# tachitachi/SR-WaveNet

Hardware: AMD Instinct MI355X
Metric: audio samples/sec (fwd+bwd) 30-layer teacher WaveNet (higher is better)
Workload: dtype bf16; 1 GPU; 30-layer teacher WaveNet (3x[1..512] dilations, 64 res / 256 skip ch, 256-way mu-law softmax), fwd+bwd+Adam, batch 8x16000 samples per GPU; global_batch=8, seq_len=16000, parallelism=dp1, launch=hipGraph

## Files before the change

include/srwn.h:

```cpp
#ifndef SRWN_H
#define SRWN_H
#include <stdint.h>

#ifdef __cplusplus
extern "C" {
#endif

#define SRWN_F32 0
#define SRWN_BF16 1

#define SRWN_E_DTYPE (-1)
#define SRWN_E_SHAPE (-2)
#define SRWN_E_NULL (-3)
#define SRWN_E_UNSUPPORTED (-4)

#define SRWN_PRO_NONE 0
#define SRWN_PRO_GATE 1
#define SRWN_EPI_NONE 0
#define SRWN_EPI_RELU 1
#define SRWN_EPI_MASK 2
#define SRWN_EPI_F32 4

int srwn_version(void);
const char* srwn_last_error(void);
// ... 80 lines not shown
                           int64_t y_row_stride, int32_t y_chunk_len, int64_t y_chunk_stride, int32_t cout_pad,
                           int32_t cout_valid, int64_t rows, int32_t dtype, void* stream);

int srwn_pw_linear_ksplit(const void* x, int64_t x_row_stride, int64_t x_chunk_stride, int32_t chunk_len, int32_t Cin,
                          const void* wpack, const float* bias, float* y_partials, int64_t y_row_stride,
                          int32_t cout_pad, int32_t cout_valid, int64_t rows, int32_t nsplit, int32_t dtype,
                          void* stream);

int64_t srwn_softmax_ce_partials(int64_t rows);
int srwn_head_softmax_ce(const void* x, int64_t x_row_stride, int32_t Cin, const void* wpack, const float* bias,
                         const int32_t* targets, float* loss_partials, void* dlogits, float* logits_out,
                         int32_t cout_pad, int32_t cout_valid, int64_t rows, float grad_scale, int32_t dtype,
                         void* stream);
int srwn_reduce_loss(const float* loss_partials, int64_t n, float scale, float* loss_out, void* stream);

int srwn_head_chain(const void* r0, const void* w1, const void* w2_perm, const void* w2T_perm, const void* w1T_perm,
                    const float* b1, const float* b2, const int32_t* targets, float* loss_partials, void* r1,
                    void* dlogits, void* da1, void* dtotal, int32_t S, int32_t cout_pad, int32_t cout_valid,
                    int64_t rows, float grad_scale, int32_t dtype, void* stream);

int srwn_residual_layer_bwd(const void* g_in, const void* df_up, const void* wconvT_up, void* g_out,
                            const void* wresT, const void* wskipT, const void* dtotal, const void* dcs,
                            const void* z, void* df_out, int32_t B, int32_t T, int32_t R, int32_t S, int32_t K,
                            int32_t dilation_up, int32_t has_up, int32_t has_down, int32_t dtype, void* stream);

int32_t srwn_wgrad_slabs(int64_t rows);
int srwn_wgrad(const void* in, int64_t in_batch_stride, int32_t cin, const void* dout, int64_t dout_batch_stride,
               int32_t cout, const void* cond, int64_t cond_batch_stride, int32_t cond_frames, int32_t pool_stride,
               int32_t cond_row_stride, const int32_t* shifts , int32_t nbatch, float* partials,
               float* bias_partials, int64_t rows, int32_t T, int32_t nslabs, int32_t pro, int32_t dtype,
               void* stream);
int srwn_reduce_partials(const float* partials, int32_t nslabs, int64_t n, int32_t nbatch, int32_t partials_batched,
                         float scale, float* out, int64_t out_batch_stride, void* stream);
#define SRWN_PARTIALS_F32 0
#define SRWN_PARTIALS_BLK16 1
#define SRWN_PARTIALS_SUM 2
typedef struct SrwnReduceJob {
  const void* partials; int32_t nslabs; int64_t n; int32_t nbatch; int32_t partials_batched; float scale;
  float* out; int64_t out_batch_stride;
  int32_t layout; int32_t blk_cols;
} SrwnReduceJob;
int srwn_reduce_partials_multi(const SrwnReduceJob* jobs, int32_t njobs, void* stream);

int srwn_add_frame_bias(void* x, const void* bias, int64_t bias_row_stride, int32_t B, int32_t T, int32_t C,
                        int32_t frames, int32_t pool_stride, int32_t dtype, void* stream);
int srwn_frame_sum(const void* g, void* out, int32_t B, int32_t T, int32_t C, int32_t frames, int32_t pool_stride,
                   int32_t dtype, void* stream);
int srwn_frame_sum_batched(const void* g, int64_t g_batch_stride, void* out, int64_t out_batch_stride, int32_t nbatch,
                           int32_t B, int32_t T, int32_t C, int32_t frames, int32_t pool_stride, float scale,
                           int32_t dtype, void* stream);

int srwn_adam_step(float* params, const float* grads, float* m, float* v, int64_t n, int64_t* step, float lr,
                   float beta1, float beta2, float eps, float grad_scale, void* stream);

int32_t srwn_time_mean_slabs(int32_t T);
int srwn_time_mean(const void* x, float* partials, float* out, int32_t B, int32_t T, int32_t C, int32_t dtype,
                   void* stream);
int srwn_pooled_head(const float* mean, const float* w2, const float* b2, const float* labels, float* probs,
                     float* loss, float* gw2, float* gb2, float* dmean, int32_t B, int32_t S, int32_t C,
                     int32_t ldw, void* stream);
int srwn_bcast_mask(const float* dmean, const void* r1, void* out, int32_t B, int32_t T, int32_t S, float scale,
                    int32_t dtype, void* stream);

int srwn_wavenet_layer_fwd(const void* x, const void* cond, const void* wconv, const void* wres, const float* bias_f,
                           const float* bias_g, const float* bias_r, void* h_out, void* z_out, void* s_out, void* c_out,
                           int32_t B, int32_t T, int32_t R, int32_t K, int32_t dilation, int32_t cond_frames,
                           int32_t pool_stride, int32_t cond_row_stride, int32_t dtype, void* stream);
int srwn_wavenet_layer_bwd(const void* g_in, const void* d_up, const void* wconvT_up, void* g_out, const void* wresT,
                           const void* wskipT, const void* dtotal, const void* dcs, const void* z, const void* s,
                           void* d_out, int32_t B, int32_t T, int32_t R, int32_t S, int32_t K, int32_t dilation_up,
                           int32_t has_up, int32_t has_down, int32_t dtype, void* stream);

int srwn_contrastive_head(const float* mean, const float* w2, const float* b2, const float* labels, float margin,
                          float* emb, float* dist, float* loss, float* gw2, float* gb2, float* dmean, int32_t rows,
                          int32_t S, int32_t D, int32_t ldw, void* stream);

int32_t srwn_wgrad256_slabs(int64_t rows, int32_t m_chunks);
int32_t srwn_wgrad_wide_slabs(int64_t rows, int32_t m_chunks, int32_t chunk_width);
int srwn_wgrad_wide(const void* a, int64_t a_chunk_stride, int64_t a_row_stride, int32_t m_chunks, int32_t chunk_width,
                    const void* d, int64_t d_row_stride, int32_t d_width, float* partials, float* bias_partials,
                    int64_t rows, int32_t nslabs, int32_t pro, int32_t dtype, void* stream);
int srwn_wgrad_wide_pair(const void* a0, const void* d0, float* partials0, float* bias_partials0, const void* a1,
                         const void* d1, float* partials1, float* bias_partials1, int64_t a_chunk_stride,
                         int64_t a_row_stride, int32_t m_chunks, int32_t chunk_width, int64_t d_row_stride,
                         int32_t d_width, int64_t rows, int32_t nslabs, int32_t pro, int32_t dtype, void* stream);
int srwn_wgrad256(const void* a, int64_t a_chunk_stride, int64_t a_row_stride, int32_t m_chunks, const void* d,
                  int64_t d_row_stride, float* partials, float* bias_partials, int64_t rows, int32_t nslabs,
                  int32_t pro, int32_t dtype, void* stream);

int srwn_skip_dgrad_all(const void* dtotal, const void* wskipT_all, void* dcs, int64_t dcs_layer_stride,
                        int32_t nlayers, int64_t rows, int32_t R, int32_t S, int32_t dtype, void* stream);

int srwn_wgrad_layers(const void* x, const void* z, const void* df, const void* g, int64_t layer_stride,
                      const void* cond, int64_t cond_layer_stride, int32_t cond_frames, int32_t pool_stride,
                      int32_t cond_row_stride, const int32_t* dilations, int32_t nlayers, float* part_f,
                      float* part_r, float* part_bf, float* part_br, int64_t rows, int32_t T, int32_t nslabs,
                      int32_t R, int32_t K, int32_t dtype, void* stream);

int32_t srwn_wgrad_skip_wt_slabs(const int32_t* st, const int32_t* seg_rows, int32_t nlayers, int32_t T);
int srwn_wgrad_skip_wt(const void* cT, int64_t wt_layer_stride, const int32_t* st, const int32_t* seg_rows,
                       int32_t nlayers, const void* d, int64_t d_row_stride, void* partials, float* bias_partials,
                       int32_t part16, int32_t nslabs, int32_t B, int32_t T, int32_t R, int32_t S, int32_t dtype,
                       void* stream);

int64_t srwn_generate_ring_elems(const int32_t* dilations, int32_t nlayers, int32_t R);
int srwn_generate(const void* wcr, const void* wskip, const void* w1, const void* w2, const float* bias_f,
// ... 323 lines not shown
```

sr-wavenet_amd/_lib.py:

```python
from __future__ import annotations

import ctypes as C
import numbers
import os

HERE = os.path.dirname(os.path.abspath(__file__))
LIB_PATH = os.path.join(HERE, "libsrwn.so")
_ALT_LIB = os.environ.get("SRWN_LIB_PATH")
if _ALT_LIB:
    LIB_PATH = _ALT_LIB

F32, BF16 = 0, 1
PRO_NONE, PRO_GATE = 0, 1
EPI_NONE, EPI_RELU, EPI_MASK, EPI_F32 = 0, 1, 2, 4

_p, _i32, _i64, _f32 = C.c_void_p, C.c_int32, C.c_int64, C.c_float


class SrwnGenSlot(C.Structure):
    _fields_ = [("t", C.c_int32), ("t_end", C.c_int32), ("seed", C.c_uint64)]


class SrwnSynthSlot(C.Structure):
    _fields_ = [("t", C.c_int64), ("t_end", C.c_int64)]
# ... 130 lines not shown
    "srwn_nc_encode_partials": (_i64, [_i32, _i32, _i32, _i32]),
    "srwn_nc_encode_frames": (C.c_int, [_p, _i64, _p, _p, _p, _p, _p, _i64, _p, _i64, _p, _p, _p, _p, _i32, _i32, _i32, _i32,
                                        _i32, _i32, _i32, _i32, _p]),
    "srwn_nc_encode_list_partials": (_i64, [_i32, _i32, _i32]),
    "srwn_nc_encode_frame_list": (C.c_int, [_p, _i32, _i32, _p, _i32, _p, _p, _p, _p, _p, _i64, _p, _i64, _p, _p, _p, _p,
                                            _i32, _i32, _i32, _i32, _i32, _p]),
    "srwn_audio_ring_put": (C.c_int, [_p, _i32, _i32, _p, _p, _p, _p, _p, _i32, _i32, _p]),
    "srwn_small_gemm": (C.c_int, [_p, _i64, _i32, _i64, _i32, _p, _i64, _i64, _i32, _i64, _p, _p, _i64, _i32, _i32,
                                  _i32, _i32, _i32, _p]),
    "srwn_small_wgrad": (C.c_int, [_p, _i64, _p, _i64, _p, _p, _i32, _i32, _i32, _f32, _p]),
    "srwn_mol_sample": (C.c_int, [_p, _i64, _i32, _p, _p, _p, _i64, _p]),
    "srwn_mol_loss_dx": (C.c_int, [_p, _i64, _p, _i32, _p, _p, _i64, _f32, _p]),
    "srwn_clamp": (C.c_int, [_p, _p, _i64, _f32, _f32, _p]),
    "srwn_clamp_bwd": (C.c_int, [_p, _p, _p, _i64, _f32, _f32, _p]),
    "srwn_flow_partials": (_i64, [_i64]),
    "srwn_flow_affine_fwd": (C.c_int, [_p, _p, _p, _p, _p, _p, _p, _i64, _i32, _i32, _p]),
    "srwn_flow_affine_bwd": (C.c_int, [_p, _p, _p, _p, _p, _f32, _p, _p, _p, _i64, _i32, _i32, _p]),
    "srwn_flow_stream_in": (C.c_int, [_p, _i64, _p, _p, _p, _p, _i32, _i32, _i64, _p, _i64, _i32, _i32, _i32, _i32, _i32,
                                      _i32, _p, _p]),
    "srwn_residual_group_fwd_stream": (C.c_int, [_p, _i64, _p, _i64, _i32, _p, _p, _p, _p, _p, _i32, _i32, _i32, _p, _i32,
                                                 _i32, _i32, _i32, _i32, _i32, _i32, _p, _p]),
    "srwn_flow_stream_out": (C.c_int, [_p, _i64, _p, _p, _p, _p, _i64, _p, _i32, _p, _i32, _i32, _i32, _i32, _i32, _i32, _p,
                                       _i32, _p]),
    "srwn_logistic_noise": (C.c_int, [_p, _i64, _p, _p, _p, _i32, _i32, _p]),
    "srwn_logistic_from_bits": (C.c_int, [_p, _p, _i64, _p]),
    "srwn_logistic_noise_slots": (C.c_int, [_p, _i64, _p, _p, _p, _i32, _i32, _p]),
    "srwn_flow_stream_in_slots": (C.c_int, [_p, _i64, _p, _p, _p, _p, _i32, _i32, _i64, _p, _i64, _i32, _i32, _i32, _i32,
                                            _i32, _i32, _p, _p]),
    "srwn_residual_group_fwd_stream_slots": (C.c_int, [_p, _i64, _p, _i64, _i32, _p, _p, _p, _p, _p, _i32, _i32, _i32, _p,
                                                       _i32, _i32, _i32, _i32, _i32, _i32, _i32, _p, _p]),
    "srwn_flow_stream_out_slots": (C.c_int, [_p, _i64, _p, _p, _p, _p, _i64, _p, _i32, _p, _i32, _i32, _i32, _i32, _i32,
                                             _i32, _p, _p, _i32, _p]),
    "srwn_flow_stream_reset_slots": (C.c_int, [_p, _i32, _p, _i32, _i64, _p, _i32, _i32, _i32, _i32, _p]),
    "srwn_cond_ring_feed": (C.c_int, [_p, _i64, _i64, _i32, _p, _p, _p, _i32, _i32, _i32, _i32, _p, _p, _p, _i32, _i32,
                                      _i32, _p]),
    "srwn_causal_conv1d_dgrad": (C.c_int, [_p, _p, _p, _i32, _i32, _i32, _i32, _i32, _i32, _i32, _i32, _f32, _i32, _p]),
    "srwn_stft_frames": (_i32, [_i32]),
    "srwn_stft_power": (C.c_int, [_p, _p, _p, _p, _i32, _i32, _p]),
    "srwn_power_loss": (C.c_int, [_p, _p, _i64, _f32, _f32, _p, _p, _p]),
    "srwn_stft_power_bwd": (C.c_int, [_p, _p, _p, _i32, _i32, _i32, _p]),
    "srwn_axpy_dev": (C.c_int, [_p, _p, _p, _f32, _i64, _p]),
    "srwn_sumsq_partials": (_i64, [_i64]),
    "srwn_sumsq": (C.c_int, [_p, _i64, _p, _p]),
    "srwn_clip_scale": (C.c_int, [_p, _i64, _f32, _f32, _p, _p]),
    "srwn_adam_step_scaled": (C.c_int, [_p, _p, _p, _p, _i64, _p, _f32, _f32, _f32, _f32, _p, _i32, _p]),
}

for _n in SAMPLED:
    SIGNATURES[_n + "_sampled"] = (SIGNATURES[_n][0], SIGNATURES[_n][1] + [_p])
del _n
for _n in ("srwn_generate", "srwn_generate16"):
    SIGNATURES[_n + "_mol_live_sampled"] = SIGNATURES[_n + "_mol_resume_sampled"]
del _n
SIGNATURES["srwn_cond_ring_scatter"] = (C.c_int, [_p, _i64, _p, _i64, _i32, _i32, _i64, _i32, _i32, _i32, _p])

_lib = None
BINDING = None


def signature_hash() -> str:
    import hashlib
    txt = ";".join("%s:%s:%s" % (n, r.__name__, ",".join(a.__name__ for a in args)) for n, (r, args) in SIGNATURES.items())
    return hashlib.sha256(txt.encode()).hexdigest()[:16]


def _address(a):
    if a is None:
        return 0
    if isinstance(a, (int, float)):
        return a
    if isinstance(a, numbers.Integral):
        return int(a)
    if isinstance(a, numbers.Real):
        return float(a)
    if isinstance(a, C.Array):
        return C.addressof(a)
    if isinstance(a, C._SimpleCData):
        return a.value or 0
    if hasattr(a, "_obj"):
        return C.addressof(a._obj)
    raise TypeError("cannot pass %r through the C-ABI" % (a,))


class _PybindLib:

    def __init__(self, mod, keepalive):
        self._keepalive = keepalive
        for name in SIGNATURES:
            fn = getattr(mod, name)
            setattr(self, name, (lambda f: lambda *args: f(*[_address(a) for a in args]))(fn))


def pybind_path() -> str:
    import sysconfig
    return os.path.join(HERE, "_srwn_pyb" + sysconfig.get_config_var("EXT_SUFFIX"))


def bind(kind: str):
    if kind not in ("pybind11", "ctypes"):
        raise RuntimeError("SRWN_BINDING=%s: pybind11 or ctypes" % kind)
    if not os.path.exists(LIB_PATH):
        raise RuntimeError(
            "libsrwn.so not found at %s: build it with `python sr-wavenet_amd/build.py` "
            "(there is no CPU fallback for the product path)" % LIB_PATH)
    if _ALT_LIB:
        kind = "ctypes"
    else:
# ... 51 lines not shown
```

sr-wavenet_amd/csrc/srwn_bwd.hip:

```cpp
#include <cstdlib>
#include "srwn_common.h"
#include "srwn_host.h"
#include "../../include/srwn.h"

using namespace srwn;

struct LayerBwdArgs {
  const void* g_in;
  const void* df_up;
  const void* wconvT;
  void* g_out;
  const void* wresT;
  const void* wskipT;
  const void* dtotal;
  const void* dcs;
  const void* z;
  void* df_out;
  int Tlen, dil_up, S, ntb, ntiles;
};

template <typename T> struct Raw4;
template <> struct Raw4<bf16_t> {
  typedef bf16x4 type;
  static __device__ __forceinline__ type load(const bf16_t* p) { return *reinterpret_cast<const bf16x4*>(p); }
  static __device__ __forceinline__ float get(const type& v, int e) { return (float)v[e]; }
};
template <> struct Raw4<float> {
  typedef f32x4 type;
  static __device__ __forceinline__ type load(const float* p) { return *reinterpret_cast<const f32x4*>(p); }
  static __device__ __forceinline__ float get(const type& v, int e) { return v[e]; }
};

template <typename T, int RT, int K, int UPM, bool GIN, bool DOWN, int SK>
__global__ __launch_bounds__(256, (sizeof(T) == 2 && SK != 0) ? 2 : 1) void layer_bwd_kernel(LayerBwdArgs a) {
  constexpr int R = 32 * RT, KS = R / 16;
  constexpr bool UP = UPM == 1, HAVEG = UPM != 0, DCS = SK == 1, LEGACY = SK == 0;
  typedef typename Raw4<T>::type raw4;
  const int KSS = a.S / 16;
  extern __shared__ __attribute__((aligned(16))) char smem[];
  Frag<T>* lds_conv = reinterpret_cast<Frag<T>*>(smem);
  Frag<T>* lds_res = lds_conv + (UP ? RT * K * KS * 64 : 0);
  Frag<T>* lds_skip = lds_res + ((HAVEG && DOWN) ? RT * KS * 64 : 0);
  const int lane = threadIdx.x & 63, wave = __builtin_amdgcn_readfirstlane(threadIdx.x >> 6);
  constexpr bool ROWS = sizeof(T) == 2 && !LEGACY;
  constexpr int LS = RowStage<T>::stride(R), VEC = RowStage<T>::VEC;
  constexpr int LPR = R / VEC, RPI = 64 / LPR, NI = 32 / RPI;
  T* stage_all = reinterpret_cast<T*>(lds_skip + ((DOWN && LEGACY) ? RT * KSS * 64 : 0));
  T* stage = stage_all + wave * (32 * LS);
  if (UP) lds_dma_copy(a.wconvT, lds_conv, RT * K * KS * 64 * (int)sizeof(Frag<T>), wave, lane, 4);
  if (HAVEG && DOWN) lds_dma_copy(a.wresT, lds_res, RT * KS * 64 * (int)sizeof(Frag<T>), wave, lane, 4);
  if (DOWN && LEGACY) lds_dma_copy(a.wskipT, lds_skip, RT * KSS * 64 * (int)sizeof(Frag<T>), wave, lane, 4);

  const int col = lane & 31, half = lane >> 5;
  struct Tile {
    raw4 gin[RT][4];
// ... 534 lines not shown
}

__global__ void reduce_partials_kernel(const float* __restrict__ partials, int nslabs, int64_t n, int nbatch,
                                       int part_batch_mul, float scale, float* __restrict__ out,
                                       int64_t out_batch_stride) {
  const int64_t i = (int64_t)blockIdx.x * blockDim.x + threadIdx.x;
  const int l = blockIdx.y;
  if (i >= n || l >= nbatch) return;
  const float* p = partials + (int64_t)l * part_batch_mul * nslabs * n + i;
  double s = 0.0;
  int k = 0;
  for (; k + 8 <= nslabs; k += 8) {
    float v[8];
#pragma unroll
    for (int j = 0; j < 8; ++j) v[j] = p[(int64_t)(k + j) * n];
#pragma unroll
    for (int j = 0; j < 8; ++j) s += (double)v[j];
  }
  for (; k < nslabs; ++k) s += (double)p[(int64_t)k * n];
  out[(int64_t)l * out_batch_stride + i] = (float)(s * (double)scale);
}

__global__ __launch_bounds__(256) void reduce_partials_wide_kernel(const float* __restrict__ partials, int nslabs,
                                                                   int64_t n, int nbatch, int part_batch_mul,
                                                                   float scale, float* __restrict__ out,
                                                                   int64_t out_batch_stride) {
  const int64_t i = (int64_t)blockIdx.x * 16 + (threadIdx.x >> 4);
  const int l = blockIdx.y, sub = threadIdx.x & 15;
  double s = 0.0;
  if (i < n) {
    const float* p = partials + (int64_t)l * part_batch_mul * nslabs * n + i;
    int k = sub;
    for (; k + 16 * 7 < nslabs; k += 16 * 8) {
      float v[8];
#pragma unroll
      for (int j = 0; j < 8; ++j) v[j] = p[(int64_t)(k + 16 * j) * n];
#pragma unroll
      for (int j = 0; j < 8; ++j) s += (double)v[j];
    }
    for (; k < nslabs; k += 16) s += (double)p[(int64_t)k * n];
  }
#pragma unroll
  for (int w = 8; w > 0; w >>= 1) s += __shfl_xor(s, w, 64);
  if (i < n && sub == 0) out[(int64_t)l * out_batch_stride + i] = (float)(s * (double)scale);
}

#define SRWN_NT_LOAD(p) __builtin_nontemporal_load(p)
constexpr int kRpMaxJobs = 16;
struct RpJob {
  const float* partials; float* out; int64_t n; int64_t out_batch_stride;
  int nslabs, nbatch, part_batch_mul; float scale; int wide; unsigned blocks_x, block0;
  int blk_cols;
  int sg;
};
struct RpMulti { RpJob j[kRpMaxJobs]; int njobs; };

__global__ __launch_bounds__(256) void reduce_partials_multi_kernel(RpMulti m) {
  int k = 0;
  while (k + 1 < m.njobs && blockIdx.x >= m.j[k + 1].block0) ++k;
  const RpJob& job = m.j[k];
  const unsigned b = blockIdx.x - job.block0;
  const unsigned bx = b % job.blocks_x;
  const int l = (int)(b / job.blocks_x);
  const int nslabs = job.nslabs;
  const int64_t n = job.n;
  if (job.wide == 4) {
    __shared__ double red[256];
    const int64_t total = (int64_t)nslabs * n;
    double acc = 0.0;
    for (int64_t i = threadIdx.x; i < total; i += 256) acc += (double)job.partials[i];
    red[threadIdx.x] = acc;
    __syncthreads();
    for (int w = 128; w > 0; w >>= 1) {
      if ((int)threadIdx.x < w) red[threadIdx.x] += red[threadIdx.x + w];
      __syncthreads();
    }
    if (threadIdx.x == 0) job.out[0] = (float)(red[0] * (double)job.scale);
    return;
  }
  if (job.wide == 3) {
    __shared__ double red[256 * 8];
    const int sg = job.sg, qpb = 256 / sg;
    const int qi = (int)threadIdx.x % qpb, g = (int)threadIdx.x / qpb;
    const int64_t q = (int64_t)bx * qpb + qi;
    const bool live = q * 8 < n;
    const int per = nslabs / sg, k0 = g * per, k1 = (g == sg - 1) ? nslabs : k0 + per;
    double s[8];
#pragma unroll
    for (int e = 0; e < 8; ++e) s[e] = 0.0;
    if (live) {
      const bf16_t* p = reinterpret_cast<const bf16_t*>(job.partials) + (int64_t)l * job.part_batch_mul * nslabs * n + q * 8;
      int k = k0;
      for (; k + 8 <= k1; k += 8) {
        srwn::bf16x8 v[8];
#pragma unroll
        for (int j = 0; j < 8; ++j) v[j] = SRWN_NT_LOAD(reinterpret_cast<const srwn::bf16x8*>(p + (int64_t)(k + j) * n));
#pragma unroll
        for (int j = 0; j < 8; ++j)
#pragma unroll
          for (int e = 0; e < 8; ++e) s[e] += (double)(float)v[j][e];
      }
      for (; k < k1; ++k) {
        const srwn::bf16x8 v = *reinterpret_cast<const srwn::bf16x8*>(p + (int64_t)k * n);
#pragma unroll
        for (int e = 0; e < 8; ++e) s[e] += (double)(float)v[e];
      }
    }
    if (sg > 1) {
      if (g > 0) {
#pragma unroll
        for (int e = 0; e < 8; ++e) red[(g * qpb + qi) * 8 + e] = s[e];
      }
      __syncthreads();
      if (g > 0) return;
      for (int gg = 1; gg < sg; ++gg) {
#pragma unroll
        for (int e = 0; e < 8; ++e) s[e] += red[(gg * qpb + qi) * 8 + e];
      }
    }
    if (!live) return;
    const int64_t blk = q >> 5;
    const int pr = (int)(q & 31);
    const int nib = job.blk_cols / 16;
    const int lane = 2 * pr;
    const int64_t row0 = 16 * (blk / nib) + 4 * (lane >> 4);
    const int col = 16 * (int)(blk % nib) + (lane & 15);
    const double sc = (double)job.scale;
    float* o = job.out + (int64_t)l * job.out_batch_stride + row0 * job.blk_cols + col;
#pragma unroll
    for (int rr = 0; rr < 4; ++rr) {
      typedef float f2 __attribute__((ext_vector_type(2)));
      *reinterpret_cast<f2*>(o + (int64_t)rr * job.blk_cols) = f2{(float)(s[rr] * sc), (float)(s[4 + rr] * sc)};
    }
  } else if (job.wide == 1) {
    const int64_t i = (int64_t)bx * 16 + (threadIdx.x >> 4);
    const int sub = threadIdx.x & 15;
    double s = 0.0;
    if (i < n) {
      const float* p = job.partials + (int64_t)l * job.part_batch_mul * nslabs * n + i;
      int q = sub;
      for (; q + 16 * 7 < nslabs; q += 16 * 8) {
        float v[8];
#pragma unroll
        for (int j = 0; j < 8; ++j) v[j] = p[(int64_t)(q + 16 * j) * n];
#pragma unroll
        for (int j = 0; j < 8; ++j) s += (double)v[j];
      }
      for (; q < nslabs; q += 16) s += (double)p[(int64_t)q * n];
    }
#pragma unroll
    for (int w = 8; w > 0; w >>= 1) s += __shfl_xor(s, w, 64);
    if (i < n && sub == 0) job.out[(int64_t)l * job.out_batch_stride + i] = (float)(s * (double)job.scale);
  } else if (job.wide == 2) {
    const int64_t i = ((int64_t)bx * 256 + threadIdx.x) * 4;
    if (i >= n) return;
    const float* p = job.partials + (int64_t)l * job.part_batch_mul * nslabs * n + i;
    double s0 = 0.0, s1 = 0.0, s2 = 0.0, s3 = 0.0;
    int q = 0;
    for (; q + 8 <= nslabs; q += 8) {
      srwn::f32x4 v[8];
#pragma unroll
      for (int j = 0; j < 8; ++j) v[j] = SRWN_NT_LOAD(reinterpret_cast<const srwn::f32x4*>(p + (int64_t)(q + j) * n));
#pragma unroll
      for (int j = 0; j < 8; ++j) { s0 += (double)v[j][0]; s1 += (double)v[j][1]; s2 += (double)v[j][2]; s3 += (double)v[j][3]; }
    }
    for (; q < nslabs; ++q) {
      const srwn::f32x4 v = *reinterpret_cast<const srwn::f32x4*>(p + (int64_t)q * n);
      s0 += (double)v[0]; s1 += (double)v[1]; s2 += (double)v[2]; s3 += (double)v[3];
    }
    const double sc = (double)job.scale;
    *reinterpret_cast<srwn::f32x4*>(job.out + (int64_t)l * job.out_batch_stride + i) =
        srwn::f32x4{(float)(s0 * sc), (float)(s1 * sc), (float)(s2 * sc), (float)(s3 * sc)};
  } else {
    const int64_t i = (int64_t)bx * 256 + threadIdx.x;
    if (i >= n) return;
    const float* p = job.partials + (int64_t)l * job.part_batch_mul * nslabs * n + i;
    double s = 0.0;
    int q = 0;
    for (; q + 8 <= nslabs; q += 8) {
      float v[8];
#pragma unroll
      for (int j = 0; j < 8; ++j) v[j] = p[(int64_t)(q + j) * n];
#pragma unroll
      for (int j = 0; j < 8; ++j) s += (double)v[j];
    }
    for (; q < nslabs; ++q) s += (double)p[(int64_t)q * n];
    job.out[(int64_t)l * job.out_batch_stride + i] = (float)(s * (double)job.scale);
  }
}

extern "C" int srwn_reduce_partials_multi(const SrwnReduceJob* jobs, int32_t njobs, void* stream) {
  if (njobs == 0) return 0;
  if (!jobs) return set_error(SRWN_E_NULL, "reduce_partials_multi: null pointer");
  if (njobs < 0 || njobs > kRpMaxJobs) return set_error(SRWN_E_SHAPE, "reduce_partials_multi: %d jobs (1..%d)", njobs, kRpMaxJobs);
  RpMulti m;
  m.njobs = 0;
  uint64_t blocks = 0;
  for (int k = 0; k < njobs; ++k) {
    const SrwnReduceJob& q = jobs[k];
    if (q.n == 0 || q.nbatch == 0) continue;
    if (!q.partials || !q.out) return set_error(SRWN_E_NULL, "reduce_partials_multi: job %d: null pointer", k);
    if (q.nslabs < 1 || q.n < 0 || q.nbatch < 0 || q.nbatch > 65535)
      return set_error(SRWN_E_SHAPE, "reduce_partials_multi: job %d: nslabs=%d n=%lld nbatch=%d", k, q.nslabs, (long long)q.n, q.nbatch);
    RpJob& j = m.j[m.njobs++];
    j.partials = reinterpret_cast<const float*>(q.partials); j.out = q.out; j.n = q.n; j.out_batch_stride = q.out_batch_stride;
    j.nslabs = q.nslabs; j.nbatch = q.nbatch; j.part_batch_mul = q.partials_batched ? 1 : 0; j.scale = q.scale;
    j.wide = (q.n <= 4096 && q.nslabs >= 32) ? 1 : 0;
    if (q.nslabs >= 128 && q.n >= 1024 && q.n % 4 == 0 && q.out_batch_stride % 4 == 0 &&
        (reinterpret_cast<uintptr_t>(q.partials) | reinterpret_cast<uintptr_t>(q.out)) % 16 == 0)
      j.wide = 2;
    j.blk_cols = 0; j.sg = 1;
    if (q.layout == SRWN_PARTIALS_BLK16) {
      if (q.blk_cols < 16 || q.blk_cols % 16 || q.n % (16 * (int64_t)q.blk_cols) || q.out_batch_stride % 2 ||
          (reinterpret_cast<uintptr_t>(q.partials) % 16) || (reinterpret_cast<uintptr_t>(q.out) % 8))
        return set_error(SRWN_E_SHAPE, "reduce_partials_multi: job %d: BLK16 layout needs n = rows*blk_cols in whole 16 x 16 blocks (n=%lld, blk_cols=%d)", k, (long long)q.n, q.blk_cols);
      j.wide = 3; j.blk_cols = q.blk_cols;
      j.sg = 1;
      while (j.sg < 8 && q.nslabs / (2 * j.sg) >= 8 && (q.n / 8) * (int64_t)q.nbatch * j.sg < (int64_t)256 * 16 * 64) j.sg *= 2;
    } else if (q.layout == SRWN_PARTIALS_SUM) {
      if (q.nbatch != 1) return set_error(SRWN_E_SHAPE, "reduce_partials_multi: job %d: SUM layout has one output", k);
      j.wide = 4;
    } else if (q.layout != SRWN_PARTIALS_F32) {
      return set_error(SRWN_E_UNSUPPORTED, "reduce_partials_multi: job %d: layout %d", k, q.layout);
    }
    j.blocks_x = (unsigned)(j.wide == 4 ? 1 : j.wide == 3 ? (q.n / 8 + 256 / j.sg - 1) / (256 / j.sg) : j.wide == 2 ? (q.n / 4 + 255) / 256 : j.wide ? (q.n + 15) / 16 : (q.n + 255) / 256);
    j.block0 = (unsigned)blocks;
    blocks += (uint64_t)j.blocks_x * (uint64_t)q.nbatch;
    if (blocks > 0x7fffffffull) return set_error(SRWN_E_SHAPE, "reduce_partials_multi: grid too large");
  }
  if (m.njobs == 0) return 0;
  hipLaunchKernelGGL(reduce_partials_multi_kernel, dim3((unsigned)blocks), dim3(256), 0, (hipStream_t)stream, m);
  return check_launch("reduce_partials_multi");
}

extern "C" int srwn_reduce_partials(const float* partials, int32_t nslabs, int64_t n, int32_t nbatch,
                                    int32_t partials_batched, float scale, float* out, int64_t out_batch_stride,
                                    void* stream) {
  if (n == 0 || nbatch == 0) return 0;
  if (!partials || !out) return set_error(SRWN_E_NULL, "reduce_partials: null pointer");
  if (nslabs < 1 || n < 0 || nbatch < 0 || nbatch > 65535) return set_error(SRWN_E_SHAPE, "reduce_partials: nslabs=%d n=%lld nbatch=%d", nslabs, (long long)n, nbatch);
  if (n <= 4096 && nslabs >= 32) {
    dim3 grid((unsigned)((n + 15) / 16), (unsigned)nbatch), block(256);
    hipLaunchKernelGGL(reduce_partials_wide_kernel, grid, block, 0, (hipStream_t)stream, partials, nslabs, n, nbatch,
                       partials_batched ? 1 : 0, scale, out, out_batch_stride);
    return check_launch("reduce_partials");
  }
  dim3 grid((unsigned)((n + 255) / 256), (unsigned)nbatch), block(256);
  hipLaunchKernelGGL(reduce_partials_kernel, grid, block, 0, (hipStream_t)stream, partials, nslabs, n, nbatch,
                     partials_batched ? 1 : 0, scale, out, out_batch_stride);
  return check_launch("reduce_partials");
}

template <typename T> struct FsRow;
template <> struct FsRow<bf16_t> {
  static __device__ __forceinline__ void load(const bf16_t* p, float (&v)[8]) {
    const bf16x8 r = *reinterpret_cast<const bf16x8*>(p);
#pragma unroll
    for (int j = 0; j < 8; ++j) v[j] = (float)r[j];
  }
};
template <> struct FsRow<float> {
  static __device__ __forceinline__ void load(const float* p, float (&v)[8]) {
    const f32x4 a = *reinterpret_cast<const f32x4*>(p), b = *reinterpret_cast<const f32x4*>(p + 4);
#pragma unroll
    for (int j = 0; j < 4; ++j) { v[j] = a[j]; v[4 + j] = b[j]; }
  }
};

template <typename T, int C>
__global__ __launch_bounds__(256) void frame_sum_kernel(const T* __restrict__ g, int64_t g_batch_stride,
                                                        T* __restrict__ out, int64_t out_batch_stride, int Tlen,
                                                        int frames, int pool, float scale) {
  constexpr int LPR = C / 8, RPI = 256 / LPR;
  __shared__ float red[256 * 8];
  const int e = blockIdx.x, b = blockIdx.y, l = blockIdx.z;
  const int sub = threadIdx.x % LPR, rloc = threadIdx.x / LPR;
  const int t0 = e * pool;
  const int t1 = min(t0 + pool, Tlen);
  const T* src = g + (int64_t)l * g_batch_stride + (int64_t)b * Tlen * C + 8 * sub;
  float acc[8] = {0, 0, 0, 0, 0, 0, 0, 0};
  for (int t = t0 + rloc; t < t1; t += RPI) {
    float v[8];
    FsRow<T>::load(src + (int64_t)t * C, v);
#pragma unroll
    for (int j = 0; j < 8; ++j) acc[j] += v[j];
// ... 108 lines not shown
```

sr-wavenet_amd/csrc/srwn_opt.hip:

```cpp
#include "srwn_common.h"
#include "srwn_host.h"
#include "../../include/srwn.h"

using namespace srwn;

constexpr int kAdamBlocks = 256;
static unsigned adam_grid(int64_t n) {
  const int64_t b = (n + 1023) / 1024;
  return (unsigned)(b < kAdamBlocks ? b : kAdamBlocks);
}
static int adam_vec(const void* a, const void* b, const void* c, const void* d) {
  return ((((uintptr_t)a) | ((uintptr_t)b) | ((uintptr_t)c) | ((uintptr_t)d)) & 15) == 0;
}

__global__ __launch_bounds__(256) void adam_step_kernel(float* __restrict__ theta, const float* __restrict__ g,
                                                        float* __restrict__ m, float* __restrict__ v, int64_t n,
                                                        int64_t* step, int tick, float lr, float b1, float b2,
                                                        float eps, float grad_scale,
                                                        const float* __restrict__ scale_dev, int vec) {
  __shared__ float s_lr;
  __shared__ int s_t;
  if (threadIdx.x == 0) {
    const int count = __hip_atomic_load(reinterpret_cast<int*>(step), __ATOMIC_RELAXED, __HIP_MEMORY_SCOPE_AGENT);
    s_t = count + (tick ? 1 : 0);
    const double t = (double)s_t;
    s_lr = (float)((double)lr * sqrt(1.0 - pow((double)b2, t)) / (1.0 - pow((double)b1, t)));
  }
  __syncthreads();
  const float lr_t = s_lr;
  if (scale_dev) grad_scale *= scale_dev[0];
  auto one = [&](float gi, float& mi, float& vi, float& th) {
    gi *= grad_scale;
    mi = b1 * mi + (1.0f - b1) * gi;
    vi = b2 * vi + (1.0f - b2) * gi * gi;
    th -= lr_t * mi / (sqrtf(vi) + eps);
  };
  for (int64_t i0 = ((int64_t)blockIdx.x * blockDim.x + threadIdx.x) * 4; i0 < n; i0 += (int64_t)gridDim.x * blockDim.x * 4) {
    if (vec && i0 + 4 <= n) {
      typedef float f4 __attribute__((ext_vector_type(4)));
      f4 gg = *reinterpret_cast<const f4*>(g + i0), mm = *reinterpret_cast<f4*>(m + i0), vv = *reinterpret_cast<f4*>(v + i0),
         tt = *reinterpret_cast<f4*>(theta + i0);
#pragma unroll
      for (int j = 0; j < 4; ++j) { float a = mm[j], b = vv[j], c = tt[j]; one(gg[j], a, b, c); mm[j] = a; vv[j] = b; tt[j] = c; }
      *reinterpret_cast<f4*>(m + i0) = mm;
      *reinterpret_cast<f4*>(v + i0) = vv;
      *reinterpret_cast<f4*>(theta + i0) = tt;
    } else {
      for (int64_t i = i0; i < n && i < i0 + 4; ++i) one(g[i], m[i], v[i], theta[i]);
    }
  }
  if (tick && threadIdx.x == 0) {
    unsigned* arrived = reinterpret_cast<unsigned*>(step) + 1;
    const unsigned prev = __hip_atomic_fetch_add(arrived, 1u, __ATOMIC_RELAXED, __HIP_MEMORY_SCOPE_AGENT);
    if (prev == gridDim.x - 1)
      __hip_atomic_store(step, (int64_t)s_t, __ATOMIC_RELAXED, __HIP_MEMORY_SCOPE_AGENT);
  }
}

extern "C" int srwn_adam_step(float* params, const float* grads, float* m, float* v, int64_t n, int64_t* step,
                              float lr, float beta1, float beta2, float eps, float grad_scale, void* stream) {
  if (n == 0) return 0;
  if (!params || !grads || !m || !v || !step) return set_error(SRWN_E_NULL, "adam_step: null pointer");
  if (n < 0) return set_error(SRWN_E_SHAPE, "adam_step: n=%lld", (long long)n);
  hipStream_t st = (hipStream_t)stream;
  hipLaunchKernelGGL(adam_step_kernel, dim3(adam_grid(n)), dim3(256), 0, st, params, grads, m, v, n,
                     step, 1, lr, beta1, beta2, eps, grad_scale, (const float*)nullptr, adam_vec(params, grads, m, v));
  return check_launch("adam_step");
}

extern "C" int srwn_adam_step_scaled(float* params, const float* grads, float* m, float* v, int64_t n, int64_t* step,
                                     float lr, float beta1, float beta2, float eps, const float* grad_scale_dev,
                                     int32_t tick, void* stream) {
  if (n == 0) return 0;
  if (!params || !grads || !m || !v || !step || !grad_scale_dev)
    return set_error(SRWN_E_NULL, "adam_step_scaled: null pointer");
  if (n < 0) return set_error(SRWN_E_SHAPE, "adam_step_scaled: n=%lld", (long long)n);
  hipStream_t st = (hipStream_t)stream;
  hipLaunchKernelGGL(adam_step_kernel, dim3(adam_grid(n)), dim3(256), 0, st, params, grads, m, v, n,
                     step, tick ? 1 : 0, lr, beta1, beta2, eps, 1.0f, grad_scale_dev, adam_vec(params, grads, m, v));
  return check_launch("adam_step_scaled");
}
```

sr-wavenet_amd/csrc/srwn_pybind.cpp:

```cpp
#include <pybind11/pybind11.h>
#include <cstdint>
#include "../../include/srwn.h"
namespace py = pybind11;
namespace {
struct P {
  std::uintptr_t v;
  template <class T> operator T*() const { return reinterpret_cast<T*>(v); }
};
}

PYBIND11_MODULE(_srwn_pyb, m) {
  m.doc() = "pybind11 binding of libsrwn.so (include/srwn.h)";
  m.attr("SIGNATURE_HASH") = "921a0d5f5da475ed";
  m.def("srwn_version", []() { return srwn_version(); });
  m.def("srwn_last_error", []() { const char* r = srwn_last_error(); return py::bytes(r ? r : ""); });
  m.def("srwn_mu_law_encode", [](std::uintptr_t a0, std::uintptr_t a1, int64_t a2, int a3, std::uintptr_t a4) { return srwn_mu_law_encode(P{a0}, P{a1}, a2, a3, P{a4}); });
  m.def("srwn_mu_law_decode", [](std::uintptr_t a0, std::uintptr_t a1, int64_t a2, int a3, std::uintptr_t a4) { return srwn_mu_law_decode(P{a0}, P{a1}, a2, a3, P{a4}); });
  m.def("srwn_pack_a_index", [](std::uintptr_t a0, int a1, int a2, int a3, int a4, int a5, int a6, int a7, int a8, int a9, int a10, std::uintptr_t a11) { return srwn_pack_a_index(P{a0}, a1, a2, a3, a4, a5, a6, a7, a8, a9, a10, P{a11}); });
  m.def("srwn_pack_gather", [](std::uintptr_t a0, std::uintptr_t a1, std::uintptr_t a2, int64_t a3, int a4, std::uintptr_t a5) { return srwn_pack_gather(P{a0}, P{a1}, P{a2}, a3, a4, P{a5}); });
  m.def("srwn_pack_gather_rowsum", [](std::uintptr_t a0, std::uintptr_t a1, std::uintptr_t a2, int64_t a3, int a4, std::uintptr_t a5, int a6, int a7, std::uintptr_t a8, std::uintptr_t a9) { return srwn_pack_gather_rowsum(P{a0}, P{a1}, P{a2}, a3, a4, P{a5}, a6, a7, P{a8}, P{a9}); });
  m.def("srwn_causal_conv1d_fwd", [](std::uintptr_t a0, std::uintptr_t a1, std::uintptr_t a2, std::uintptr_t a3, int a4, int a5, int a6, int a7, int a8, int a9, int a10, int a11, std::uintptr_t a12) { return srwn_causal_conv1d_fwd(P{a0}, P{a1}, P{a2}, P{a3}, a4, a5, a6, a7, a8, a9, a10, a11, P{a12}); });
  m.def("srwn_init_conv_wgrad_partials", [](int a0, int a1, int a2, int a3) { return srwn_init_conv_wgrad_partials(a0, a1, a2, a3); });
  m.def("srwn_init_conv_wgrad", [](std::uintptr_t a0, std::uintptr_t a1, std::uintptr_t a2, std::uintptr_t a3, std::uintptr_t a4, int a5, int a6, int a7, int a8, int a9, int a10, std::uintptr_t a11) { return srwn_init_conv_wgrad(P{a0}, P{a1}, P{a2}, P{a3}, P{a4}, a5, a6, a7, a8, a9, a10, P{a11}); });
  m.def("srwn_residual_layer_fwd", [](std::uintptr_t a0, std::uintptr_t a1, std::uintptr_t a2, std::uintptr_t a3, std::uintptr_t a4, std::uintptr_t a5, std::uintptr_t a6, std::uintptr_t a7, int a8, int a9, int a10, int a11, int a12, int a13, int a14, int a15, int a16, std::uintptr_t a17) { return srwn_residual_layer_fwd(P{a0}, P{a1}, P{a2}, P{a3}, P{a4}, P{a5}, P{a6}, P{a7}, a8, a9, a10, a11, a12, a13, a14, a15, a16, P{a17}); });
  m.def("srwn_residual_group_fwd", [](std::uintptr_t a0, std::uintptr_t a1, std::uintptr_t a2, int64_t a3, std::uintptr_t a4, std::uintptr_t a5, std::uintptr_t a6, std::uintptr_t a7, std::uintptr_t a8, int a9, int a10, int a11, std::uintptr_t a12, int a13, int a14, int a15, int a16, int a17, int a18, int a19, std::uintptr_t a20) { return srwn_residual_group_fwd(P{a0}, P{a1}, P{a2}, a3, P{a4}, P{a5}, P{a6}, P{a7}, P{a8}, a9, a10, a11, P{a12}, a13, a14, a15, a16, a17, a18, a19, P{a20}); });
  m.def("srwn_residual_group_bwd", [](std::uintptr_t a0, std::uintptr_t a1, std::uintptr_t a2, std::uintptr_t a3, std::uintptr_t a4, int64_t a5, std::uintptr_t a6, std::uintptr_t a7, std::uintptr_t a8, int a9, int a10, int a11, int a12, int a13, int a14, int a15, std::uintptr_t a16) { return srwn_residual_group_bwd(P{a0}, P{a1}, P{a2}, P{a3}, P{a4}, a5, P{a6}, P{a7}, P{a8}, a9, a10, a11, a12, a13, a14, a15, P{a16}); });
  m.def("srwn_group_wt_geometry", [](std::uintptr_t a0, int a1, int a2, int a3, int a4, int a5, int a6, std::uintptr_t a7, std::uintptr_t a8, std::uintptr_t a9, std::uintptr_t a10) { return srwn_group_wt_geometry(P{a0}, a1, a2, a3, a4, a5, a6, P{a7}, P{a8}, P{a9}, P{a10}); });
  m.def("srwn_residual_group_fwd_wt", [](std::uintptr_t a0, std::uintptr_t a1, std::uintptr_t a2, int64_t a3, std::uintptr_t a4, std::uintptr_t a5, int64_t a6, int a7, std::uintptr_t a8, std::uintptr_t a9, std::uintptr_t a10, std::uintptr_t a11, std::uintptr_t a12, int a13, int a14, int a15, std::uintptr_t a16, int a17, int a18, int a19, int a20, int a21, int a22, int a23, std::uintptr_t a24) { return srwn_residual_group_fwd_wt(P{a0}, P{a1}, P{a2}, a3, P{a4}, P{a5}, a6, a7, P{a8}, P{a9}, P{a10}, P{a11}, P{a12}, a13, a14, a15, P{a16}, a17, a18, a19, a20, a21, a22, a23, P{a24}); });
  m.def("srwn_residual_group_fwd_ic", [](std::uintptr_t a0, std::uintptr_t a1, std::uintptr_t a2, int a3, std::uintptr_t a4, std::uintptr_t a5, int64_t a6, std::uintptr_t a7, std::uintptr_t a8, int64_t a9, int a10, std::uintptr_t a11, std::uintptr_t a12, std::uintptr_t a13, std::uintptr_t a14, std::uintptr_t a15, int a16, int a17, int a18, int a19, int a20, int a21, int a22, std::uintptr_t a23) { return srwn_residual_group_fwd_ic(P{a0}, P{a1}, P{a2}, a3, P{a4}, P{a5}, a6, P{a7}, P{a8}, a9, a10, P{a11}, P{a12}, P{a13}, P{a14}, P{a15}, a16, a17, a18, a19, a20, a21, a22, P{a23}); });
  m.def("srwn_residual_group_bwd_wt", [](std::uintptr_t a0, std::uintptr_t a1, int a2, std::uintptr_t a3, std::uintptr_t a4, int64_t a5, std::uintptr_t a6, std::uintptr_t a7, int64_t a8, std::uintptr_t a9, std::uintptr_t a10, std::uintptr_t a11, int a12, std::uintptr_t a13, std::uintptr_t a14, std::uintptr_t a15, std::uintptr_t a16, int a17, std::uintptr_t a18, std::uintptr_t a19, int a20, int a21, int a22, int a23, int a24, int a25, int a26, int a27, std::uintptr_t a28) { return srwn_residual_group_bwd_wt(P{a0}, P{a1}, a2, P{a3}, P{a4}, a5, P{a6}, P{a7}, a8, P{a9}, P{a10}, P{a11}, a12, P{a13}, P{a14}, P{a15}, P{a16}, a17, P{a18}, P{a19}, a20, a21, a22, a23, a24, a25, a26, a27, P{a28}); });
  m.def("srwn_debug_stamp_buffer", [](std::uintptr_t a0) { return srwn_debug_stamp_buffer(P{a0}); });
  m.def("srwn_group_plan_auto", [](std::uintptr_t a0, int a1, int a2, int a3, int a4, int a5, int a6, std::uintptr_t a7) { return srwn_group_plan_auto(P{a0}, a1, a2, a3, a4, a5, a6, P{a7}); });
  m.def("srwn_log_softmax", [](std::uintptr_t a0, std::uintptr_t a1, std::uintptr_t a2, int64_t a3, int a4, std::uintptr_t a5) { return srwn_log_softmax(P{a0}, P{a1}, P{a2}, a3, a4, P{a5}); });
  m.def("srwn_categorical_sample", [](std::uintptr_t a0, std::uintptr_t a1, int64_t a2, int a3, uint64_t a4, std::uintptr_t a5) { return srwn_categorical_sample(P{a0}, P{a1}, a2, a3, a4, P{a5}); });
  m.def("srwn_probs_logistic", [](std::uintptr_t a0, std::uintptr_t a1, std::uintptr_t a2, std::uintptr_t a3, int64_t a4, int a5, float a6, std::uintptr_t a7) { return srwn_probs_logistic(P{a0}, P{a1}, P{a2}, P{a3}, a4, a5, a6, P{a7}); });
  m.def("srwn_tanh_gate", [](std::uintptr_t a0, std::uintptr_t a1, std::uintptr_t a2, int64_t a3, std::uintptr_t a4) { return srwn_tanh_gate(P{a0}, P{a1}, P{a2}, a3, P{a4}); });
  m.def("srwn_gated_activation", [](std::uintptr_t a0, std::uintptr_t a1, std::uintptr_t a2, std::uintptr_t a3, int64_t a4, int a5, std::uintptr_t a6) { return srwn_gated_activation(P{a0}, P{a1}, P{a2}, P{a3}, a4, a5, P{a6}); });
  m.def("srwn_residual_combine", [](std::uintptr_t a0, int a1, std::uintptr_t a2, int a3, std::uintptr_t a4, int64_t a5, std::uintptr_t a6) { return srwn_residual_combine(P{a0}, a1, P{a2}, a3, P{a4}, a5, P{a6}); });
  m.def("srwn_relu", [](std::uintptr_t a0, std::uintptr_t a1, int64_t a2, std::uintptr_t a3) { return srwn_relu(P{a0}, P{a1}, a2, P{a3}); });
  m.def("srwn_mol_nll_rows", [](std::uintptr_t a0, int64_t a1, std::uintptr_t a2, int a3, std::uintptr_t a4, int64_t a5, std::uintptr_t a6) { return srwn_mol_nll_rows(P{a0}, a1, P{a2}, a3, P{a4}, a5, P{a6}); });
  m.def("srwn_group_plan", [](std::uintptr_t a0, int a1, int a2, int a3, std::uintptr_t a4) { return srwn_group_plan(P{a0}, a1, a2, a3, P{a4}); });
  m.def("srwn_pw_linear_ychunks", [](std::uintptr_t a0, int64_t a1, int a2, std::uintptr_t a3, std::uintptr_t a4, std::uintptr_t a5, int64_t a6, int a7, int64_t a8, int a9, int a10, int64_t a11, int a12, std::uintptr_t a13) { return srwn_pw_linear_ychunks(P{a0}, a1, a2, P{a3}, P{a4}, P{a5}, a6, a7, a8, a9, a10, a11, a12, P{a13}); });
  m.def("srwn_pw_linear", [](std::uintptr_t a0, int64_t a1, int64_t a2, int a3, int a4, std::uintptr_t a5, std::uintptr_t a6, std::uintptr_t a7, int64_t a8, int a9, int a10, int64_t a11, std::uintptr_t a12, int64_t a13, int a14, int a15, int a16, std::uintptr_t a17) { return srwn_pw_linear(P{a0}, a1, a2, a3, a4, P{a5}, P{a6}, P{a7}, a8, a9, a10, a11, P{a12}, a13, a14, a15, a16, P{a17}); });
  m.def("srwn_pw_linear_ksplit", [](std::uintptr_t a0, int64_t a1, int64_t a2, int a3, int a4, std::uintptr_t a5, std::uintptr_t a6, std::uintptr_t a7, int64_t a8, int a9, int a10, int64_t a11, int a12, int a13, std::uintptr_t a14) { return srwn_pw_linear_ksplit(P{a0}, a1, a2, a3, a4, P{a5}, P{a6}, P{a7}, a8, a9, a10, a11, a12, a13, P{a14}); });
  m.def("srwn_softmax_ce_partials", [](int64_t a0) { return srwn_softmax_ce_partials(a0); });
  m.def("srwn_head_softmax_ce", [](std::uintptr_t a0, int64_t a1, int a2, std::uintptr_t a3, std::uintptr_t a4, std::uintptr_t a5, std::uintptr_t a6, std::uintptr_t a7, std::uintptr_t a8, int a9, int a10, int64_t a11, float a12, int a13, std::uintptr_t a14) { return srwn_head_softmax_ce(P{a0}, a1, a2, P{a3}, P{a4}, P{a5}, P{a6}, P{a7}, P{a8}, a9, a10, a11, a12, a13, P{a14}); });
  m.def("srwn_reduce_loss", [](std::uintptr_t a0, int64_t a1, float a2, std::uintptr_t a3, std::uintptr_t a4) { return srwn_reduce_loss(P{a0}, a1, a2, P{a3}, P{a4}); });
  m.def("srwn_head_chain", [](std::uintptr_t a0, std::uintptr_t a1, std::uintptr_t a2, std::uintptr_t a3, std::uintptr_t a4, std::uintptr_t a5, std::uintptr_t a6, std::uintptr_t a7, std::uintptr_t a8, std::uintptr_t a9, std::uintptr_t a10, std::uintptr_t a11, std::uintptr_t a12, int a13, int a14, int a15, int64_t a16, float a17, int a18, std::uintptr_t a19) { return srwn_head_chain(P{a0}, P{a1}, P{a2}, P{a3}, P{a4}, P{a5}, P{a6}, P{a7}, P{a8}, P{a9}, P{a10}, P{a11}, P{a12}, a13, a14, a15, a16, a17, a18, P{a19}); });
  m.def("srwn_residual_layer_bwd", [](std::uintptr_t a0, std::uintptr_t a1, std::uintptr_t a2, std::uintptr_t a3, std::uintptr_t a4, std::uintptr_t a5, std::uintptr_t a6, std::uintptr_t a7, std::uintptr_t a8, std::uintptr_t a9, int a10, int a11, int a12, int a13, int a14, int a15, int a16, int a17, int a18, std::uintptr_t a19) { return srwn_residual_layer_bwd(P{a0}, P{a1}, P{a2}, P{a3}, P{a4}, P{a5}, P{a6}, P{a7}, P{a8}, P{a9}, a10, a11, a12, a13, a14, a15, a16, a17, a18, P{a19}); });
  m.def("srwn_wgrad_slabs", [](int64_t a0) { return srwn_wgrad_slabs(a0); });
  m.def("srwn_wgrad", [](std::uintptr_t a0, int64_t a1, int a2, std::uintptr_t a3, int64_t a4, int a5, std::uintptr_t a6, int64_t a7, int a8, int a9, int a10, std::uintptr_t a11, int a12, std::uintptr_t a13, std::uintptr_t a14, int64_t a15, int a16, int a17, int a18, int a19, std::uintptr_t a20) { return srwn_wgrad(P{a0}, a1, a2, P{a3}, a4, a5, P{a6}, a7, a8, a9, a10, P{a11}, a12, P{a13}, P{a14}, a15, a16, a17, a18, a19, P{a20}); });
  m.def("srwn_reduce_partials", [](std::uintptr_t a0, int a1, int64_t a2, int a3, int a4, float a5, std::uintptr_t a6, int64_t a7, std::uintptr_t a8) { return srwn_reduce_partials(P{a0}, a1, a2, a3, a4, a5, P{a6}, a7, P{a8}); });
  m.def("srwn_reduce_partials_multi", [](std::uintptr_t a0, int a1, std::uintptr_t a2) { return srwn_reduce_partials_multi(P{a0}, a1, P{a2}); });
  m.def("srwn_add_frame_bias", [](std::uintptr_t a0, std::uintptr_t a1, int64_t a2, int a3, int a4, int a5, int a6, int a7, int a8, std::uintptr_t a9) { return srwn_add_frame_bias(P{a0}, P{a1}, a2, a3, a4, a5, a6, a7, a8, P{a9}); });
  m.def("srwn_frame_sum", [](std::uintptr_t a0, std::uintptr_t a1, int a2, int a3, int a4, int a5, int a6, int a7, std::uintptr_t a8) { return srwn_frame_sum(P{a0}, P{a1}, a2, a3, a4, a5, a6, a7, P{a8}); });
  m.def("srwn_frame_sum_batched", [](std::uintptr_t a0, int64_t a1, std::uintptr_t a2, int64_t a3, int a4, int a5, int a6, int a7, int a8, int a9, float a10, int a11, std::uintptr_t a12) { return srwn_frame_sum_batched(P{a0}, a1, P{a2}, a3, a4, a5, a6, a7, a8, a9, a10, a11, P{a12}); });
  m.def("srwn_adam_step", [](std::uintptr_t a0, std::uintptr_t a1, std::uintptr_t a2, std::uintptr_t a3, int64_t a4, std::uintptr_t a5, float a6, float a7, float a8, float a9, float a10, std::uintptr_t a11) { return srwn_adam_step(P{a0}, P{a1}, P{a2}, P{a3}, a4, P{a5}, a6, a7, a8, a9, a10, P{a11}); });
  m.def("srwn_time_mean_slabs", [](int a0) { return srwn_time_mean_slabs(a0); });
  m.def("srwn_time_mean", [](std::uintptr_t a0, std::uintptr_t a1, std::uintptr_t a2, int a3, int a4, int a5, int a6, std::uintptr_t a7) { return srwn_time_mean(P{a0}, P{a1}, P{a2}, a3, a4, a5, a6, P{a7}); });
  m.def("srwn_pooled_head", [](std::uintptr_t a0, std::uintptr_t a1, std::uintptr_t a2, std::uintptr_t a3, std::uintptr_t a4, std::uintptr_t a5, std::uintptr_t a6, std::uintptr_t a7, std::uintptr_t a8, int a9, int a10, int a11, int a12, std::uintptr_t a13) { return srwn_pooled_head(P{a0}, P{a1}, P{a2}, P{a3}, P{a4}, P{a5}, P{a6}, P{a7}, P{a8}, a9, a10, a11, a12, P{a13}); });
  m.def("srwn_bcast_mask", [](std::uintptr_t a0, std::uintptr_t a1, std::uintptr_t a2, int a3, int a4, int a5, float a6, int a7, std::uintptr_t a8) { return srwn_bcast_mask(P{a0}, P{a1}, P{a2}, a3, a4, a5, a6, a7, P{a8}); });
  m.def("srwn_contrastive_head", [](std::uintptr_t a0, std::uintptr_t a1, std::uintptr_t a2, std::uintptr_t a3, float a4, std::uintptr_t a5, std::uintptr_t a6, std::uintptr_t a7, std::uintptr_t a8, std::uintptr_t a9, std::uintptr_t a10, int a11, int a12, int a13, int a14, std::uintptr_t a15) { return srwn_contrastive_head(P{a0}, P{a1}, P{a2}, P{a3}, a4, P{a5}, P{a6}, P{a7}, P{a8}, P{a9}, P{a10}, a11, a12, a13, a14, P{a15}); });
  m.def("srwn_wavenet_layer_fwd", [](std::uintptr_t a0, std::uintptr_t a1, std::uintptr_t a2, std::uintptr_t a3, std::uintptr_t a4, std::uintptr_t a5, std::uintptr_t a6, std::uintptr_t a7, std::uintptr_t a8, std::uintptr_t a9, std::uintptr_t a10, int a11, int a12, int a13, int a14, int a15, int a16, int a17, int a18, int a19, std::uintptr_t a20) { return srwn_wavenet_layer_fwd(P{a0}, P{a1}, P{a2}, P{a3}, P{a4}, P{a5}, P{a6}, P{a7}, P{a8}, P{a9}, P{a10}, a11, a12, a13, a14, a15, a16, a17, a18, a19, P{a20}); });
  m.def("srwn_wavenet_layer_bwd", [](std::uintptr_t a0, std::uintptr_t a1, std::uintptr_t a2, std::uintptr_t a3, std::uintptr_t a4, std::uintptr_t a5, std::uintptr_t a6, std::uintptr_t a7, std::uintptr_t a8, std::uintptr_t a9, std::uintptr_t a10, int a11, int a12, int a13, int a14, int a15, int a16, int a17, int a18, int a19, std::uintptr_t a20) { return srwn_wavenet_layer_bwd(P{a0}, P{a1}, P{a2}, P{a3}, P{a4}, P{a5}, P{a6}, P{a7}, P{a8}, P{a9}, P{a10}, a11, a12, a13, a14, a15, a16, a17, a18, a19, P{a20}); });
  m.def("srwn_skip_dgrad_all", [](std::uintptr_t a0, std::uintptr_t a1, std::uintptr_t a2, int64_t a3, int a4, int64_t a5, int a6, int a7, int a8, std::uintptr_t a9) { return srwn_skip_dgrad_all(P{a0}, P{a1}, P{a2}, a3, a4, a5, a6, a7, a8, P{a9}); });
  m.def("srwn_wgrad_layers", [](std::uintptr_t a0, std::uintptr_t a1, std::uintptr_t a2, std::uintptr_t a3, int64_t a4, std::uintptr_t a5, int64_t a6, int a7, int a8, int a9, std::uintptr_t a10, int a11, std::uintptr_t a12, std::uintptr_t a13, std::uintptr_t a14, std::uintptr_t a15, int64_t a16, int a17, int a18, int a19, int a20, int a21, std::uintptr_t a22) { return srwn_wgrad_layers(P{a0}, P{a1}, P{a2}, P{a3}, a4, P{a5}, a6, a7, a8, a9, P{a10}, a11, P{a12}, P{a13}, P{a14}, P{a15}, a16, a17, a18, a19, a20, a21, P{a22}); });
// ... 25 lines not shown
  m.def("srwn_tap_linear", [](std::uintptr_t a0, int64_t a1, int a2, int a3, int a4, int a5, std::uintptr_t a6, std::uintptr_t a7, std::uintptr_t a8, int64_t a9, int a10, int64_t a11, std::uintptr_t a12, int64_t a13, std::uintptr_t a14, int64_t a15, int a16, int a17, float a18, int a19, int a20, std::uintptr_t a21) { return srwn_tap_linear(P{a0}, a1, a2, a3, a4, a5, P{a6}, P{a7}, P{a8}, a9, a10, a11, P{a12}, a13, P{a14}, a15, a16, a17, a18, a19, a20, P{a21}); });
  m.def("srwn_wgrad_nc_layers", [](std::uintptr_t a0, std::uintptr_t a1, std::uintptr_t a2, std::uintptr_t a3, int64_t a4, int a5, std::uintptr_t a6, std::uintptr_t a7, std::uintptr_t a8, std::uintptr_t a9, int64_t a10, int a11, int a12, int a13, int a14, int a15, std::uintptr_t a16) { return srwn_wgrad_nc_layers(P{a0}, P{a1}, P{a2}, P{a3}, a4, a5, P{a6}, P{a7}, P{a8}, P{a9}, a10, a11, a12, a13, a14, a15, P{a16}); });
  m.def("srwn_nc_input_fwd", [](std::uintptr_t a0, std::uintptr_t a1, std::uintptr_t a2, std::uintptr_t a3, int a4, int a5, int a6, int a7, int a8, std::uintptr_t a9) { return srwn_nc_input_fwd(P{a0}, P{a1}, P{a2}, P{a3}, a4, a5, a6, a7, a8, P{a9}); });
  m.def("srwn_nc_layer_fwd", [](std::uintptr_t a0, std::uintptr_t a1, std::uintptr_t a2, std::uintptr_t a3, std::uintptr_t a4, std::uintptr_t a5, std::uintptr_t a6, std::uintptr_t a7, std::uintptr_t a8, int a9, int a10, int a11, int a12, int a13, std::uintptr_t a14) { return srwn_nc_layer_fwd(P{a0}, P{a1}, P{a2}, P{a3}, P{a4}, P{a5}, P{a6}, P{a7}, P{a8}, a9, a10, a11, a12, a13, P{a14}); });
  m.def("srwn_nc_mask_words", [](int a0, int a1) { return srwn_nc_mask_words(a0, a1); });
  m.def("srwn_nc_mask_bits", [](std::uintptr_t a0, std::uintptr_t a1, int a2, int a3, int a4, int a5, std::uintptr_t a6) { return srwn_nc_mask_bits(P{a0}, P{a1}, a2, a3, a4, a5, P{a6}); });
  m.def("srwn_nc_layer_bwd", [](std::uintptr_t a0, std::uintptr_t a1, std::uintptr_t a2, std::uintptr_t a3, std::uintptr_t a4, std::uintptr_t a5, int64_t a6, int a7, int a8, float a9, std::uintptr_t a10, std::uintptr_t a11, int a12, int a13, int a14, int a15, int a16, std::uintptr_t a17) { return srwn_nc_layer_bwd(P{a0}, P{a1}, P{a2}, P{a3}, P{a4}, P{a5}, a6, a7, a8, a9, P{a10}, P{a11}, a12, a13, a14, a15, a16, P{a17}); });
  m.def("srwn_nc_encode_max_layers", []() { return srwn_nc_encode_max_layers(); });
  m.def("srwn_nc_encode_partials", [](int a0, int a1, int a2, int a3) { return srwn_nc_encode_partials(a0, a1, a2, a3); });
  m.def("srwn_nc_encode_frames", [](std::uintptr_t a0, int64_t a1, std::uintptr_t a2, std::uintptr_t a3, std::uintptr_t a4, std::uintptr_t a5, std::uintptr_t a6, int64_t a7, std::uintptr_t a8, int64_t a9, std::uintptr_t a10, std::uintptr_t a11, std::uintptr_t a12, std::uintptr_t a13, int a14, int a15, int a16, int a17, int a18, int a19, int a20, int a21, std::uintptr_t a22) { return srwn_nc_encode_frames(P{a0}, a1, P{a2}, P{a3}, P{a4}, P{a5}, P{a6}, a7, P{a8}, a9, P{a10}, P{a11}, P{a12}, P{a13}, a14, a15, a16, a17, a18, a19, a20, a21, P{a22}); });
  m.def("srwn_nc_encode_list_partials", [](int a0, int a1, int a2) { return srwn_nc_encode_list_partials(a0, a1, a2); });
  m.def("srwn_nc_encode_frame_list", [](std::uintptr_t a0, int a1, int a2, std::uintptr_t a3, int a4, std::uintptr_t a5, std::uintptr_t a6, std::uintptr_t a7, std::uintptr_t a8, std::uintptr_t a9, int64_t a10, std::uintptr_t a11, int64_t a12, std::uintptr_t a13, std::uintptr_t a14, std::uintptr_t a15, std::uintptr_t a16, int a17, int a18, int a19, int a20, int a21, std::uintptr_t a22) { return srwn_nc_encode_frame_list(P{a0}, a1, a2, P{a3}, a4, P{a5}, P{a6}, P{a7}, P{a8}, P{a9}, a10, P{a11}, a12, P{a13}, P{a14}, P{a15}, P{a16}, a17, a18, a19, a20, a21, P{a22}); });
  m.def("srwn_audio_ring_put", [](std::uintptr_t a0, int a1, int a2, std::uintptr_t a3, std::uintptr_t a4, std::uintptr_t a5, std::uintptr_t a6, std::uintptr_t a7, int a8, int a9, std::uintptr_t a10) { return srwn_audio_ring_put(P{a0}, a1, a2, P{a3}, P{a4}, P{a5}, P{a6}, P{a7}, a8, a9, P{a10}); });
  m.def("srwn_small_gemm", [](std::uintptr_t a0, int64_t a1, int a2, int64_t a3, int a4, std::uintptr_t a5, int64_t a6, int64_t a7, int a8, int64_t a9, std::uintptr_t a10, std::uintptr_t a11, int64_t a12, int a13, int a14, int a15, int a16, int a17, std::uintptr_t a18) { return srwn_small_gemm(P{a0}, a1, a2, a3, a4, P{a5}, a6, a7, a8, a9, P{a10}, P{a11}, a12, a13, a14, a15, a16, a17, P{a18}); });
  m.def("srwn_small_wgrad", [](std::uintptr_t a0, int64_t a1, std::uintptr_t a2, int64_t a3, std::uintptr_t a4, std::uintptr_t a5, int a6, int a7, int a8, float a9, std::uintptr_t a10) { return srwn_small_wgrad(P{a0}, a1, P{a2}, a3, P{a4}, P{a5}, a6, a7, a8, a9, P{a10}); });
  m.def("srwn_mol_sample", [](std::uintptr_t a0, int64_t a1, int a2, std::uintptr_t a3, std::uintptr_t a4, std::uintptr_t a5, int64_t a6, std::uintptr_t a7) { return srwn_mol_sample(P{a0}, a1, a2, P{a3}, P{a4}, P{a5}, a6, P{a7}); });
  m.def("srwn_mol_loss_dx", [](std::uintptr_t a0, int64_t a1, std::uintptr_t a2, int a3, std::uintptr_t a4, std::uintptr_t a5, int64_t a6, float a7, std::uintptr_t a8) { return srwn_mol_loss_dx(P{a0}, a1, P{a2}, a3, P{a4}, P{a5}, a6, a7, P{a8}); });
  m.def("srwn_clamp", [](std::uintptr_t a0, std::uintptr_t a1, int64_t a2, float a3, float a4, std::uintptr_t a5) { return srwn_clamp(P{a0}, P{a1}, a2, a3, a4, P{a5}); });
  m.def("srwn_clamp_bwd", [](std::uintptr_t a0, std::uintptr_t a1, std::uintptr_t a2, int64_t a3, float a4, float a5, std::uintptr_t a6) { return srwn_clamp_bwd(P{a0}, P{a1}, P{a2}, a3, a4, a5, P{a6}); });
  m.def("srwn_flow_partials", [](int64_t a0) { return srwn_flow_partials(a0); });
  m.def("srwn_flow_affine_fwd", [](std::uintptr_t a0, std::uintptr_t a1, std::uintptr_t a2, std::uintptr_t a3, std::uintptr_t a4, std::uintptr_t a5, std::uintptr_t a6, int64_t a7, int a8, int a9, std::uintptr_t a10) { return srwn_flow_affine_fwd(P{a0}, P{a1}, P{a2}, P{a3}, P{a4}, P{a5}, P{a6}, a7, a8, a9, P{a10}); });
  m.def("srwn_flow_affine_bwd", [](std::uintptr_t a0, std::uintptr_t a1, std::uintptr_t a2, std::uintptr_t a3, std::uintptr_t a4, float a5, std::uintptr_t a6, std::uintptr_t a7, std::uintptr_t a8, int64_t a9, int a10, int a11, std::uintptr_t a12) { return srwn_flow_affine_bwd(P{a0}, P{a1}, P{a2}, P{a3}, P{a4}, a5, P{a6}, P{a7}, P{a8}, a9, a10, a11, P{a12}); });
  m.def("srwn_flow_stream_in", [](std::uintptr_t a0, int64_t a1, std::uintptr_t a2, std::uintptr_t a3, std::uintptr_t a4, std::uintptr_t a5, int a6, int a7, int64_t a8, std::uintptr_t a9, int64_t a10, int a11, int a12, int a13, int a14, int a15, int a16, std::uintptr_t a17, std::uintptr_t a18) { return srwn_flow_stream_in(P{a0}, a1, P{a2}, P{a3}, P{a4}, P{a5}, a6, a7, a8, P{a9}, a10, a11, a12, a13, a14, a15, a16, P{a17}, P{a18}); });
  m.def("srwn_residual_group_fwd_stream", [](std::uintptr_t a0, int64_t a1, std::uintptr_t a2, int64_t a3, int a4, std::uintptr_t a5, std::uintptr_t a6, std::uintptr_t a7, std::uintptr_t a8, std::uintptr_t a9, int a10, int a11, int a12, std::uintptr_t a13, int a14, int a15, int a16, int a17, int a18, int a19, int a20, std::uintptr_t a21, std::uintptr_t a22) { return srwn_residual_group_fwd_stream(P{a0}, a1, P{a2}, a3, a4, P{a5}, P{a6}, P{a7}, P{a8}, P{a9}, a10, a11, a12, P{a13}, a14, a15, a16, a17, a18, a19, a20, P{a21}, P{a22}); });
  m.def("srwn_flow_stream_out", [](std::uintptr_t a0, int64_t a1, std::uintptr_t a2, std::uintptr_t a3, std::uintptr_t a4, std::uintptr_t a5, int64_t a6, std::uintptr_t a7, int a8, std::uintptr_t a9, int a10, int a11, int a12, int a13, int a14, int a15, std::uintptr_t a16, int a17, std::uintptr_t a18) { return srwn_flow_stream_out(P{a0}, a1, P{a2}, P{a3}, P{a4}, P{a5}, a6, P{a7}, a8, P{a9}, a10, a11, a12, a13, a14, a15, P{a16}, a17, P{a18}); });
  m.def("srwn_logistic_noise", [](std::uintptr_t a0, int64_t a1, std::uintptr_t a2, std::uintptr_t a3, std::uintptr_t a4, int a5, int a6, std::uintptr_t a7) { return srwn_logistic_noise(P{a0}, a1, P{a2}, P{a3}, P{a4}, a5, a6, P{a7}); });
  m.def("srwn_logistic_from_bits", [](std::uintptr_t a0, std::uintptr_t a1, int64_t a2, std::uintptr_t a3) { return srwn_logistic_from_bits(P{a0}, P{a1}, a2, P{a3}); });
  m.def("srwn_logistic_noise_slots", [](std::uintptr_t a0, int64_t a1, std::uintptr_t a2, std::uintptr_t a3, std::uintptr_t a4, int a5, int a6, std::uintptr_t a7) { return srwn_logistic_noise_slots(P{a0}, a1, P{a2}, P{a3}, P{a4}, a5, a6, P{a7}); });
  m.def("srwn_flow_stream_in_slots", [](std::uintptr_t a0, int64_t a1, std::uintptr_t a2, std::uintptr_t a3, std::uintptr_t a4, std::uintptr_t a5, int a6, int a7, int64_t a8, std::uintptr_t a9, int64_t a10, int a11, int a12, int a13, int a14, int a15, int a16, std::uintptr_t a17, std::uintptr_t a18) { return srwn_flow_stream_in_slots(P{a0}, a1, P{a2}, P{a3}, P{a4}, P{a5}, a6, a7, a8, P{a9}, a10, a11, a12, a13, a14, a15, a16, P{a17}, P{a18}); });
  m.def("srwn_residual_group_fwd_stream_slots", [](std::uintptr_t a0, int64_t a1, std::uintptr_t a2, int64_t a3, int a4, std::uintptr_t a5, std::uintptr_t a6, std::uintptr_t a7, std::uintptr_t a8, std::uintptr_t a9, int a10, int a11, int a12, std::uintptr_t a13, int a14, int a15, int a16, int a17, int a18, int a19, int a20, std::uintptr_t a21, std::uintptr_t a22) { return srwn_residual_group_fwd_stream_slots(P{a0}, a1, P{a2}, a3, a4, P{a5}, P{a6}, P{a7}, P{a8}, P{a9}, a10, a11, a12, P{a13}, a14, a15, a16, a17, a18, a19, a20, P{a21}, P{a22}); });
  m.def("srwn_flow_stream_out_slots", [](std::uintptr_t a0, int64_t a1, std::uintptr_t a2, std::uintptr_t a3, std::uintptr_t a4, std::uintptr_t a5, int64_t a6, std::uintptr_t a7, int a8, std::uintptr_t a9, int a10, int a11, int a12, int a13, int a14, int a15, std::uintptr_t a16, std::uintptr_t a17, int a18, std::uintptr_t a19) { return srwn_flow_stream_out_slots(P{a0}, a1, P{a2}, P{a3}, P{a4}, P{a5}, a6, P{a7}, a8, P{a9}, a10, a11, a12, a13, a14, a15, P{a16}, P{a17}, a18, P{a19}); });
  m.def("srwn_flow_stream_reset_slots", [](std::uintptr_t a0, int a1, std::uintptr_t a2, int a3, int64_t a4, std::uintptr_t a5, int a6, int a7, int a8, int a9, std::uintptr_t a10) { return srwn_flow_stream_reset_slots(P{a0}, a1, P{a2}, a3, a4, P{a5}, a6, a7, a8, a9, P{a10}); });
  m.def("srwn_cond_ring_feed", [](std::uintptr_t a0, int64_t a1, int64_t a2, int a3, std::uintptr_t a4, std::uintptr_t a5, std::uintptr_t a6, int a7, int a8, int a9, int a10, std::uintptr_t a11, std::uintptr_t a12, std::uintptr_t a13, int a14, int a15, int a16, std::uintptr_t a17) { return srwn_cond_ring_feed(P{a0}, a1, a2, a3, P{a4}, P{a5}, P{a6}, a7, a8, a9, a10, P{a11}, P{a12}, P{a13}, a14, a15, a16, P{a17}); });
  m.def("srwn_causal_conv1d_dgrad", [](std::uintptr_t a0, std::uintptr_t a1, std::uintptr_t a2, int a3, int a4, int a5, int a6, int a7, int a8, int a9, int a10, float a11, int a12, std::uintptr_t a13) { return srwn_causal_conv1d_dgrad(P{a0}, P{a1}, P{a2}, a3, a4, a5, a6, a7, a8, a9, a10, a11, a12, P{a13}); });
  m.def("srwn_stft_frames", [](int a0) { return srwn_stft_frames(a0); });
  m.def("srwn_stft_power", [](std::uintptr_t a0, std::uintptr_t a1, std::uintptr_t a2, std::uintptr_t a3, int a4, int a5, std::uintptr_t a6) { return srwn_stft_power(P{a0}, P{a1}, P{a2}, P{a3}, a4, a5, P{a6}); });
  m.def("srwn_power_loss", [](std::uintptr_t a0, std::uintptr_t a1, int64_t a2, float a3, float a4, std::uintptr_t a5, std::uintptr_t a6, std::uintptr_t a7) { return srwn_power_loss(P{a0}, P{a1}, a2, a3, a4, P{a5}, P{a6}, P{a7}); });
  m.def("srwn_stft_power_bwd", [](std::uintptr_t a0, std::uintptr_t a1, std::uintptr_t a2, int a3, int a4, int a5, std::uintptr_t a6) { return srwn_stft_power_bwd(P{a0}, P{a1}, P{a2}, a3, a4, a5, P{a6}); });
  m.def("srwn_axpy_dev", [](std::uintptr_t a0, std::uintptr_t a1, std::uintptr_t a2, float a3, int64_t a4, std::uintptr_t a5) { return srwn_axpy_dev(P{a0}, P{a1}, P{a2}, a3, a4, P{a5}); });
  m.def("srwn_sumsq_partials", [](int64_t a0) { return srwn_sumsq_partials(a0); });
  m.def("srwn_sumsq", [](std::uintptr_t a0, int64_t a1, std::uintptr_t a2, std::uintptr_t a3) { return srwn_sumsq(P{a0}, a1, P{a2}, P{a3}); });
  m.def("srwn_clip_scale", [](std::uintptr_t a0, int64_t a1, float a2, float a3, std::uintptr_t a4, std::uintptr_t a5) { return srwn_clip_scale(P{a0}, a1, a2, a3, P{a4}, P{a5}); });
  m.def("srwn_adam_step_scaled", [](std::uintptr_t a0, std::uintptr_t a1, std::uintptr_t a2, std::uintptr_t a3, int64_t a4, std::uintptr_t a5, float a6, float a7, float a8, float a9, std::uintptr_t a10, int a11, std::uintptr_t a12) { return srwn_adam_step_scaled(P{a0}, P{a1}, P{a2}, P{a3}, a4, P{a5}, a6, a7, a8, a9, P{a10}, a11, P{a12}); });
  m.def("srwn_generate_resume_sampled", [](std::uintptr_t a0, std::uintptr_t a1, std::uintptr_t a2, std::uintptr_t a3, std::uintptr_t a4, std::uintptr_t a5, std::uintptr_t a6, std::uintptr_t a7, std::uintptr_t a8, std::uintptr_t a9, std::uintptr_t a10, std::uintptr_t a11, std::uintptr_t a12, std::uintptr_t a13, std::uintptr_t a14, std::uintptr_t a15, std::uintptr_t a16, int a17, int a18, int a19, int a20, int a21, int a22, int a23, int a24, int a25, uint64_t a26, int a27, std::uintptr_t a28, int a29, std::uintptr_t a30, std::uintptr_t a31) { return srwn_generate_resume_sampled(P{a0}, P{a1}, P{a2}, P{a3}, P{a4}, P{a5}, P{a6}, P{a7}, P{a8}, P{a9}, P{a10}, P{a11}, P{a12}, P{a13}, P{a14}, P{a15}, P{a16}, a17, a18, a19, a20, a21, a22, a23, a24, a25, a26, a27, P{a28}, a29, P{a30}, P{a31}); });
  m.def("srwn_generate_mol_resume_sampled", [](std::uintptr_t a0, std::uintptr_t a1, std::uintptr_t a2, std::uintptr_t a3, std::uintptr_t a4, std::uintptr_t a5, std::uintptr_t a6, std::uintptr_t a7, std::uintptr_t a8, std::uintptr_t a9, std::uintptr_t a10, std::uintptr_t a11, std::uintptr_t a12, std::uintptr_t a13, std::uintptr_t a14, std::uintptr_t a15, std::uintptr_t a16, int a17, int a18, int a19, int a20, int a21, int a22, int a23, int a24, std::uintptr_t a25, int a26, int a27, int64_t a28, int a29, uint64_t a30, int a31, std::uintptr_t a32, int a33, std::uintptr_t a34, std::uintptr_t a35) { return srwn_generate_mol_resume_sampled(P{a0}, P{a1}, P{a2}, P{a3}, P{a4}, P{a5}, P{a6}, P{a7}, P{a8}, P{a9}, P{a10}, P{a11}, P{a12}, P{a13}, P{a14}, P{a15}, P{a16}, a17, a18, a19, a20, a21, a22, a23, a24, P{a25}, a26, a27, a28, a29, a30, a31, P{a32}, a33, P{a34}, P{a35}); });
  m.def("srwn_generate16_resume_sampled", [](std::uintptr_t a0, std::uintptr_t a1, std::uintptr_t a2, std::uintptr_t a3, std::uintptr_t a4, std::uintptr_t a5, std::uintptr_t a6, std::uintptr_t a7, std::uintptr_t a8, std::uintptr_t a9, std::uintptr_t a10, std::uintptr_t a11, std::uintptr_t a12, std::uintptr_t a13, std::uintptr_t a14, std::uintptr_t a15, int a16, int a17, int a18, int a19, int a20, int a21, int a22, int a23, uint64_t a24, std::uintptr_t a25, int a26, std::uintptr_t a27, std::uintptr_t a28) { return srwn_generate16_resume_sampled(P{a0}, P{a1}, P{a2}, P{a3}, P{a4}, P{a5}, P{a6}, P{a7}, P{a8}, P{a9}, P{a10}, P{a11}, P{a12}, P{a13}, P{a14}, P{a15}, a16, a17, a18, a19, a20, a21, a22, a23, a24, P{a25}, a26, P{a27}, P{a28}); });
  m.def("srwn_generate16_mol_resume_sampled", [](std::uintptr_t a0, std::uintptr_t a1, std::uintptr_t a2, std::uintptr_t a3, std::uintptr_t a4, std::uintptr_t a5, std::uintptr_t a6, std::uintptr_t a7, std::uintptr_t a8, std::uintptr_t a9, std::uintptr_t a10, std::uintptr_t a11, std::uintptr_t a12, std::uintptr_t a13, std::uintptr_t a14, std::uintptr_t a15, int a16, int a17, int a18, int a19, int a20, int a21, int a22, std::uintptr_t a23, int a24, int a25, int64_t a26, int a27, uint64_t a28, std::uintptr_t a29, int a30, std::uintptr_t a31, std::uintptr_t a32) { return srwn_generate16_mol_resume_sampled(P{a0}, P{a1}, P{a2}, P{a3}, P{a4}, P{a5}, P{a6}, P{a7}, P{a8}, P{a9}, P{a10}, P{a11}, P{a12}, P{a13}, P{a14}, P{a15}, a16, a17, a18, a19, a20, a21, a22, P{a23}, a24, a25, a26, a27, a28, P{a29}, a30, P{a31}, P{a32}); });
  m.def("srwn_generate_slots_sampled", [](std::uintptr_t a0, std::uintptr_t a1, std::uintptr_t a2, std::uintptr_t a3, std::uintptr_t a4, std::uintptr_t a5, std::uintptr_t a6, std::uintptr_t a7, std::uintptr_t a8, std::uintptr_t a9, std::uintptr_t a10, std::uintptr_t a11, std::uintptr_t a12, std::uintptr_t a13, std::uintptr_t a14, std::uintptr_t a15, std::uintptr_t a16, int a17, int a18, int a19, int a20, int a21, int a22, int a23, int a24, int a25, int a26, std::uintptr_t a27, int a28, std::uintptr_t a29, std::uintptr_t a30, std::uintptr_t a31) { return srwn_generate_slots_sampled(P{a0}, P{a1}, P{a2}, P{a3}, P{a4}, P{a5}, P{a6}, P{a7}, P{a8}, P{a9}, P{a10}, P{a11}, P{a12}, P{a13}, P{a14}, P{a15}, P{a16}, a17, a18, a19, a20, a21, a22, a23, a24, a25, a26, P{a27}, a28, P{a29}, P{a30}, P{a31}); });
  m.def("srwn_generate_mol_slots_sampled", [](std::uintptr_t a0, std::uintptr_t a1, std::uintptr_t a2, std::uintptr_t a3, std::uintptr_t a4, std::uintptr_t a5, std::uintptr_t a6, std::uintptr_t a7, std::uintptr_t a8, std::uintptr_t a9, std::uintptr_t a10, std::uintptr_t a11, std::uintptr_t a12, std::uintptr_t a13, std::uintptr_t a14, std::uintptr_t a15, std::uintptr_t a16, int a17, int a18, int a19, int a20, int a21, int a22, int a23, int a24, std::uintptr_t a25, int a26, int a27, int64_t a28, int a29, int a30, std::uintptr_t a31, int a32, std::uintptr_t a33, std::uintptr_t a34, std::uintptr_t a35) { return srwn_generate_mol_slots_sampled(P{a0}, P{a1}, P{a2}, P{a3}, P{a4}, P{a5}, P{a6}, P{a7}, P{a8}, P{a9}, P{a10}, P{a11}, P{a12}, P{a13}, P{a14}, P{a15}, P{a16}, a17, a18, a19, a20, a21, a22, a23, a24, P{a25}, a26, a27, a28, a29, a30, P{a31}, a32, P{a33}, P{a34}, P{a35}); });
  m.def("srwn_generate16_slots_sampled", [](std::uintptr_t a0, std::uintptr_t a1, std::uintptr_t a2, std::uintptr_t a3, std::uintptr_t a4, std::uintptr_t a5, std::uintptr_t a6, std::uintptr_t a7, std::uintptr_t a8, std::uintptr_t a9, std::uintptr_t a10, std::uintptr_t a11, std::uintptr_t a12, std::uintptr_t a13, std::uintptr_t a14, std::uintptr_t a15, int a16, int a17, int a18, int a19, int a20, int a21, int a22, int a23, std::uintptr_t a24, int a25, std::uintptr_t a26, std::uintptr_t a27, std::uintptr_t a28) { return srwn_generate16_slots_sampled(P{a0}, P{a1}, P{a2}, P{a3}, P{a4}, P{a5}, P{a6}, P{a7}, P{a8}, P{a9}, P{a10}, P{a11}, P{a12}, P{a13}, P{a14}, P{a15}, a16, a17, a18, a19, a20, a21, a22, a23, P{a24}, a25, P{a26}, P{a27}, P{a28}); });
  m.def("srwn_generate16_mol_slots_sampled", [](std::uintptr_t a0, std::uintptr_t a1, std::uintptr_t a2, std::uintptr_t a3, std::uintptr_t a4, std::uintptr_t a5, std::uintptr_t a6, std::uintptr_t a7, std::uintptr_t a8, std::uintptr_t a9, std::uintptr_t a10, std::uintptr_t a11, std::uintptr_t a12, std::uintptr_t a13, std::uintptr_t a14, std::uintptr_t a15, int a16, int a17, int a18, int a19, int a20, int a21, int a22, std::uintptr_t a23, int a24, int a25, int64_t a26, int a27, std::uintptr_t a28, int a29, std::uintptr_t a30, std::uintptr_t a31, std::uintptr_t a32) { return srwn_generate16_mol_slots_sampled(P{a0}, P{a1}, P{a2}, P{a3}, P{a4}, P{a5}, P{a6}, P{a7}, P{a8}, P{a9}, P{a10}, P{a11}, P{a12}, P{a13}, P{a14}, P{a15}, a16, a17, a18, a19, a20, a21, a22, P{a23}, a24, a25, a26, a27, P{a28}, a29, P{a30}, P{a31}, P{a32}); });
  m.def("srwn_generate_mol_live_sampled", [](std::uintptr_t a0, std::uintptr_t a1, std::uintptr_t a2, std::uintptr_t a3, std::uintptr_t a4, std::uintptr_t a5, std::uintptr_t a6, std::uintptr_t a7, std::uintptr_t a8, std::uintptr_t a9, std::uintptr_t a10, std::uintptr_t a11, std::uintptr_t a12, std::uintptr_t a13, std::uintptr_t a14, std::uintptr_t a15, std::uintptr_t a16, int a17, int a18, int a19, int a20, int a21, int a22, int a23, int a24, std::uintptr_t a25, int a26, int a27, int64_t a28, int a29, uint64_t a30, int a31, std::uintptr_t a32, int a33, std::uintptr_t a34, std::uintptr_t a35) { return srwn_generate_mol_live_sampled(P{a0}, P{a1}, P{a2}, P{a3}, P{a4}, P{a5}, P{a6}, P{a7}, P{a8}, P{a9}, P{a10}, P{a11}, P{a12}, P{a13}, P{a14}, P{a15}, P{a16}, a17, a18, a19, a20, a21, a22, a23, a24, P{a25}, a26, a27, a28, a29, a30, a31, P{a32}, a33, P{a34}, P{a35}); });
  m.def("srwn_generate16_mol_live_sampled", [](std::uintptr_t a0, std::uintptr_t a1, std::uintptr_t a2, std::uintptr_t a3, std::uintptr_t a4, std::uintptr_t a5, std::uintptr_t a6, std::uintptr_t a7, std::uintptr_t a8, std::uintptr_t a9, std::uintptr_t a10, std::uintptr_t a11, std::uintptr_t a12, std::uintptr_t a13, std::uintptr_t a14, std::uintptr_t a15, int a16, int a17, int a18, int a19, int a20, int a21, int a22, std::uintptr_t a23, int a24, int a25, int64_t a26, int a27, uint64_t a28, std::uintptr_t a29, int a30, std::uintptr_t a31, std::uintptr_t a32) { return srwn_generate16_mol_live_sampled(P{a0}, P{a1}, P{a2}, P{a3}, P{a4}, P{a5}, P{a6}, P{a7}, P{a8}, P{a9}, P{a10}, P{a11}, P{a12}, P{a13}, P{a14}, P{a15}, a16, a17, a18, a19, a20, a21, a22, P{a23}, a24, a25, a26, a27, a28, P{a29}, a30, P{a31}, P{a32}); });
  m.def("srwn_cond_ring_scatter", [](std::uintptr_t a0, int64_t a1, std::uintptr_t a2, int64_t a3, int a4, int a5, int64_t a6, int a7, int a8, int a9, std::uintptr_t a10) { return srwn_cond_ring_scatter(P{a0}, a1, P{a2}, a3, a4, a5, a6, a7, a8, a9, P{a10}); });
}
```

sr-wavenet_amd/csrc/srwn_util.hip:

```cpp
#include "srwn_common.h"
#include "srwn_host.h"
#include "../../include/srwn.h"

using namespace srwn;

static thread_local char g_err[512] = "";
namespace srwn {
int set_error(int code, const char* fmt, ...) {
  va_list ap;
  va_start(ap, fmt);
  vsnprintf(g_err, sizeof(g_err), fmt, ap);
  va_end(ap);
  return code;
}
int check_launch(const char* what) {
  hipError_t e = hipGetLastError();
  if (e != hipSuccess) return set_error((int)e, "%s: %s", what, hipGetErrorString(e));
  return 0;
}
}

extern "C" int srwn_version(void) { return 112; }
extern "C" const char* srwn_last_error(void) { return g_err; }

__global__ void mu_law_encode_kernel(const float* __restrict__ audio, int32_t* __restrict__ codes, int64_t n,
                                     float mu, float log1p_mu) {
  int64_t i = (int64_t)blockIdx.x * blockDim.x + threadIdx.x;
  if (i >= n) return;
  float a = audio[i];
  float safe = fminf(fabsf(a), 1.0f);
  float lm = (float)log1p((double)__fmul_rn(mu, safe));
  float magnitude = __fdiv_rn(lm, log1p_mu);
  float sgn = (a > 0.0f) ? 1.0f : ((a < 0.0f) ? -1.0f : 0.0f);
  float signal = __fmul_rn(sgn, magnitude);
  float q = __fadd_rn(__fmul_rn(__fdiv_rn(__fadd_rn(signal, 1.0f), 2.0f), mu), 0.5f);
  codes[i] = (int32_t)q;
}

__global__ void mu_law_decode_kernel(const int32_t* __restrict__ codes, float* __restrict__ audio, int64_t n,
                                     float mu, float inv_mu, double base) {
  int64_t i = (int64_t)blockIdx.x * blockDim.x + threadIdx.x;
  if (i >= n) return;
  float o = (float)codes[i];
  float signal = __fadd_rn(__fmul_rn(2.0f, __fdiv_rn(o, mu)), -1.0f);
  float p = (float)pow(base, (double)fabsf(signal));
  float magnitude = __fmul_rn(inv_mu, __fadd_rn(p, -1.0f));
  float sgn = (signal > 0.0f) ? 1.0f : ((signal < 0.0f) ? -1.0f : 0.0f);
  audio[i] = __fmul_rn(sgn, magnitude);
}

extern "C" int srwn_mu_law_encode(const float* audio, int32_t* codes, int64_t n, int32_t Q, void* stream) {
  if (n == 0) return 0;
  if (!audio || !codes) return set_error(SRWN_E_NULL, "mu_law_encode: null pointer");
  if (n < 0 || Q < 2) return set_error(SRWN_E_SHAPE, "mu_law_encode: n=%lld Q=%d", (long long)n, Q);
  float mu = (float)(Q - 1);
  float l1p = (float)log1p((double)mu);
  hipLaunchKernelGGL(mu_law_encode_kernel, dim3((unsigned)((n + 255) / 256)), dim3(256), 0, (hipStream_t)stream,
                     audio, codes, n, mu, l1p);
  return check_launch("mu_law_encode");
}

extern "C" int srwn_mu_law_decode(const int32_t* codes, float* audio, int64_t n, int32_t Q, void* stream) {
  if (n == 0) return 0;
  if (!audio || !codes) return set_error(SRWN_E_NULL, "mu_law_decode: null pointer");
  if (n < 0 || Q < 2) return set_error(SRWN_E_SHAPE, "mu_law_decode: n=%lld Q=%d", (long long)n, Q);
  int mu = Q - 1;
  hipLaunchKernelGGL(mu_law_decode_kernel, dim3((unsigned)((n + 255) / 256)), dim3(256), 0, (hipStream_t)stream,
                     codes, audio, n, (float)mu, (float)(1.0 / (double)mu), (double)(1 + mu));
  return check_launch("mu_law_decode");
}

__global__ void pack_a_index_kernel(int32_t* __restrict__ dst, int32_t src_offset, int32_t rows_valid,
                                    int32_t k_valid, int32_t row_stride, int32_t k_stride, int32_t mt_count,
                                    int32_t ks_total, int32_t ks_offset, int32_t ks_count, int32_t perm_from_ks) {
  int64_t i = (int64_t)blockIdx.x * blockDim.x + threadIdx.x;
  int64_t total = (int64_t)mt_count * ks_count * 64 * 8;
  if (i >= total) return;
  int j = (int)(i & 7);
  int lane = (int)((i >> 3) & 63);
  int ksl = (int)((i >> 9) % ks_count);
  int mt = (int)((i >> 9) / ks_count);
  int r = lane & 31, h = lane >> 5;
  int kin = (ksl >= perm_from_ks) ? (8 * (j >> 2) + 4 * h + (j & 3)) : (8 * h + j);
  int k = 16 * ksl + kin;
  int row = 32 * mt + r;
  int32_t v = (row < rows_valid && k < k_valid) ? (src_offset + row * row_stride + k * k_stride) : -1;
  int64_t o = ((((int64_t)mt * ks_total + (ks_offset + ksl)) * 64) + lane) * 8 + j;
  dst[o] = v;
}

extern "C" int srwn_pack_a_index(int32_t* dst_idx, int32_t src_offset, int32_t rows_valid, int32_t k_valid,
                                 int32_t row_stride, int32_t k_stride, int32_t mt_count, int32_t ks_total,
                                 int32_t ks_offset, int32_t ks_count, int32_t perm_from_ks, void* stream) {
  if (!dst_idx) return set_error(SRWN_E_NULL, "pack_a_index: null dst");
  if (mt_count <= 0 || ks_count <= 0 || ks_offset < 0 || ks_offset + ks_count > ks_total)
    return set_error(SRWN_E_SHAPE, "pack_a_index: mt=%d ks=[%d,+%d) of %d", mt_count, ks_offset, ks_count, ks_total);
  int64_t total = (int64_t)mt_count * ks_count * 512;
  hipLaunchKernelGGL(pack_a_index_kernel, dim3((unsigned)((total + 255) / 256)), dim3(256), 0, (hipStream_t)stream,
                     dst_idx, src_offset, rows_valid, k_valid, row_stride, k_stride, mt_count, ks_total, ks_offset,
                     ks_count, perm_from_ks);
  return check_launch("pack_a_index");
}

template <typename T>
__global__ __launch_bounds__(256) void pack_gather_kernel(const float* __restrict__ src, const int32_t* __restrict__ idx,
                                                          T* __restrict__ dst, int64_t n, unsigned gather_blocks,
                                                          const float* __restrict__ sum_src, int sum_rows, int sum_cols,
                                                          float* __restrict__ sum_out) {
  if (blockIdx.x >= gather_blocks) {
    const int c = (int)(blockIdx.x - gather_blocks) * 256 + (int)threadIdx.x;
    if (c < sum_cols) {
      double s = 0.0;
      for (int l = 0; l < sum_rows; ++l) s += (double)sum_src[(size_t)l * sum_cols + c];
      sum_out[c] = (float)s;
    }
    return;
  }
  const int64_t i0 = ((int64_t)blockIdx.x * blockDim.x + threadIdx.x) * 8;
  if (i0 >= n) return;
  if (i0 + 8 <= n) {
    typedef int i32x4 __attribute__((ext_vector_type(4)));
    const i32x4 a = *reinterpret_cast<const i32x4*>(idx + i0), b = *reinterpret_cast<const i32x4*>(idx + i0 + 4);
    float v[8];
#pragma unroll
    for (int j = 0; j < 4; ++j) { v[j] = a[j] >= 0 ? src[a[j]] : 0.0f; v[4 + j] = b[j] >= 0 ? src[b[j]] : 0.0f; }
    if constexpr (sizeof(T) == 2) {
      bf16x8 o;
#pragma unroll
      for (int j = 0; j < 8; ++j) o[j] = (bf16_t)v[j];
      *reinterpret_cast<bf16x8*>(dst + i0) = o;
    } else {
      *reinterpret_cast<f32x4*>(dst + i0) = f32x4{v[0], v[1], v[2], v[3]};
      *reinterpret_cast<f32x4*>(dst + i0 + 4) = f32x4{v[4], v[5], v[6], v[7]};
    }
  } else {
    for (int64_t i = i0; i < n; ++i) {
      const int32_t s = idx[i];
      dst[i] = (T)(s >= 0 ? src[s] : 0.0f);
    }
  }
}

extern "C" int srwn_pack_gather_rowsum(const float* src, const int32_t* idx, void* dst, int64_t n, int32_t dtype,
                                       const float* sum_src, int32_t sum_rows, int32_t sum_cols, float* sum_out,
                                       void* stream) {
  const bool sum = sum_rows > 0 && sum_cols > 0;
  if (n == 0 && !sum) return 0;
  if (n < 0 || sum_rows < 0 || sum_cols < 0) return set_error(SRWN_E_SHAPE, "pack_gather: n=%lld sum %d x %d", (long long)n, sum_rows, sum_cols);
  if (n > 0 && (!src || !idx || !dst)) return set_error(SRWN_E_NULL, "pack_gather: null pointer");
  if (sum && (!sum_src || !sum_out)) return set_error(SRWN_E_NULL, "pack_gather_rowsum: null pointer");
  if (((uintptr_t)idx | (uintptr_t)dst) & 15) return set_error(SRWN_E_SHAPE, "pack_gather: idx and dst must be 16-byte aligned");
  const unsigned gb = (unsigned)((n + 2047) / 2048), sb = sum ? (unsigned)((sum_cols + 255) / 256) : 0u;
  dim3 grid(gb + sb), block(256);
  if (dtype == SRWN_F32)
    hipLaunchKernelGGL(pack_gather_kernel<float>, grid, block, 0, (hipStream_t)stream, src, idx, (float*)dst, n, gb, sum_src,
                       sum ? sum_rows : 0, sum ? sum_cols : 0, sum_out);
  else if (dtype == SRWN_BF16)
    hipLaunchKernelGGL(pack_gather_kernel<bf16_t>, grid, block, 0, (hipStream_t)stream, src, idx, (bf16_t*)dst, n, gb, sum_src,
                       sum ? sum_rows : 0, sum ? sum_cols : 0, sum_out);
  else
    return set_error(SRWN_E_DTYPE, "pack_gather: dtype %d", dtype);
  return check_launch("pack_gather");
}

extern "C" int srwn_pack_gather(const float* src, const int32_t* idx, void* dst, int64_t n, int32_t dtype,
                                void* stream) {
  return srwn_pack_gather_rowsum(src, idx, dst, n, dtype, nullptr, 0, 0, nullptr, stream);
}

template <typename TOut>
__global__ void causal_conv_kernel(const float* __restrict__ x, const float* __restrict__ w,
                                   const float* __restrict__ bias, TOut* __restrict__ y, int B, int T, int Cin,
                                   int Cout, int K, int dilation, int shift) {
  int64_t i = (int64_t)blockIdx.x * blockDim.x + threadIdx.x;
  int cq = (Cout + 3) / 4;
  int64_t total = (int64_t)B * T * cq;
  if (i >= total) return;
  int o0 = (int)(i % cq) * 4;
  int64_t bt = i / cq;
  int t = (int)(bt % T);
  int b = (int)(bt / T);
  float acc[4];
#pragma unroll
  for (int q = 0; q < 4; ++q) acc[q] = (bias && o0 + q < Cout) ? bias[o0 + q] : 0.0f;
  for (int k = 0; k < K; ++k) {
    int tk = t - (K - 1 - k) * dilation - shift;
    if (tk < 0 || tk >= T) continue;
    const float* xr = x + ((int64_t)b * T + tk) * Cin;
    const float* wk = w + (int64_t)k * Cin * Cout;
    for (int ci = 0; ci < Cin; ++ci) {
      float xv = xr[ci];
#pragma unroll
      for (int q = 0; q < 4; ++q)
// ... 232 lines not shown
```

sr-wavenet_amd/engine.py:

```python
from __future__ import annotations

import ctypes
import math
import os as _os
from dataclasses import dataclass, field
from typing import Dict, List, Optional, Sequence, Tuple

import numpy as np
import torch

from . import dp
from . import kernels as K
from . import packing as P

SQRT_HALF = 0.7071067811865476


@dataclass
class StackConfig:
    dilations: Sequence[int]
    filter_width: int = 2
    dilation_channels: int = 32
    skip_channels: int = 256
    output_channels: int = 256
# ... 312 lines not shown

CONTRASTIVE_LDS_FLOATS = 65536 // 4


class WaveNetEngine:
    def __init__(self, cfg: StackConfig, batch: int, length: int, device="cuda", seed: int = 0,
                 process_group=None, share_from: Optional["WaveNetEngine"] = None, frozen: bool = False):
        if cfg.gate_mode not in ("reference", "wavenet"):
            raise ValueError("gate_mode %r: 'reference' or 'wavenet'" % (cfg.gate_mode,))
        if cfg.gate_mode == "wavenet" and cfg.head_mode == "flow":
            raise NotImplementedError("gate_mode 'wavenet' is not built for the flows of ParallelWaveNet")
        if cfg.filter_width != 2:
            raise NotImplementedError("filter_width %d: only 2 is built (reference default, model.py:9)" % cfg.filter_width)
        if cfg.dilation_channels not in (32, 64):
            raise NotImplementedError("dilation_channels %d: built for 32 and 64" % cfg.dilation_channels)
        if cfg.skip_channels % 32 or cfg.skip_channels < 32:
            raise NotImplementedError("skip_channels must be a multiple of 32")
        if cfg.output_channels < 1 or cfg.output_channels > 256:
            raise NotImplementedError("output_channels must be in [1, 256]")
        if cfg.head_mode == "mol" and (cfg.output_channels % 4 or not 4 <= cfg.output_channels <= 64):
            raise ValueError("mol head: output_channels = 4 * num_mixtures (<= 16 mixtures)")
        if cfg.head_mode not in ("per_timestep", "pooled", "mol", "flow", "contrastive"):
            raise ValueError("head_mode %r" % cfg.head_mode)
        if cfg.head_mode == "contrastive":
            need = batch * cfg.output_channels + (batch if batch % 2 == 0 else 0)
            if need > CONTRASTIVE_LDS_FLOATS:
                raise ValueError("contrastive head: B=%d clips x D=%d dimensions (+ 2 per pair) need %d floats, over the "
                                 "head kernel's limit of %d (64 KiB of LDS)"
                                 % (batch, cfg.output_channels, need, CONTRASTIVE_LDS_FLOATS))
        if cfg.cond_channels and (length % cfg.pool_stride):
            raise ValueError("length %d is not a multiple of pool_stride %d" % (length, cfg.pool_stride))
        self.cfg = cfg
        self.wavenet = cfg.gate_mode == "wavenet"
        self.timing = False
        self.timing_overlap = False
        self.spans: Dict[str, list] = {}
        import os as _os
        fuse = _os.environ.get("SRWN_FUSE", "1")
        self.fuse_fwd = fuse not in ("0", "bwd") and not self.wavenet
        self.fuse_bwd = fuse not in ("0", "fwd") and not self.wavenet
        self.fuse_wt = _os.environ.get("SRWN_FUSE_WT", "1") != "0"
        self.wt_store_x = _os.environ.get("SRWN_WT_STORE_X", "0") != "0"
        self.fuse_ic = _os.environ.get("SRWN_FUSE_IC", "1") != "0"
        self.frozen = bool(frozen)
        self._tiles_valid = False
        will_group = (self.fuse_bwd and cfg.dilation_channels in (32, 64) and cfg.filter_width == 2 and
                      ((cfg.dilation_channels, cfg.skip_channels) in ((64, 256), (32, 128)) or cfg.head_mode == "flow"))
        self.overlap = _os.environ.get("SRWN_OVERLAP", "0" if will_group else "1") != "0"
        self.seg_rows = int(_os.environ.get("SRWN_SEG_ROWS", "0"))
        self.head_chain = (_os.environ.get("SRWN_HEAD_CHAIN", "1") != "0" and cfg.head_mode == "per_timestep"
                           and cfg.dtype == torch.bfloat16 and cfg.skip_channels == 256)
        self._head_bwd_done = False
        self._ic_job = None
        self._loss_job = None
        self.defer_loss = _os.environ.get("SRWN_DEFER_LOSS", "1") != "0"
        self.side = None
        if torch.cuda.is_available() and self.overlap:
            self.side = torch.cuda.Stream(priority=0)
        self.B, self.T = int(batch), int(length)
        self.N = self.B * self.T
        self.L = len(cfg.dilations)
        self.dil = [int(d) for d in cfg.dilations]
        self.R, self.S, self.C = cfg.dilation_channels, cfg.skip_channels, cfg.output_channels
        self.Kw = cfg.filter_width
        self.Cp = (self.C + 31) // 32 * 32
        self.E = cfg.cond_channels
        self.Ep = (self.E + 15) // 16 * 16
        self.frames = self.T // cfg.pool_stride if self.E else 0
        self.dev = torch.device(device)
        self.dt = cfg.dtype
        gl = int(_os.environ.get("SRWN_GROUP_LAYERS", "8"))
        if _os.environ.get("SRWN_GROUP_PLAN", "greedy") == "auto" and self.R in (32, 64):
            self.groups = K.group_plan_auto(self.dil, self.B, self.T, self.R, self.dt, gl)
        else:
            self.groups = K.group_plan(self.dil, 31, gl)
        self.pg = process_group
        self.world = dp.world_size(process_group)
        if share_from is None:
            self._build_params(seed)
            self._build_packing()
        else:
            for a in ("sections", "nparams", "params", "grads", "adam_m", "adam_v", "adam_step", "bs_sum", "dead_gate",
                      "packer", "packed", "pack_train_elems", "o_conv", "o_res", "o_convT", "o_resT", "o_skipT", "o_skipT_all", "o_skip", "o_gen", "o_skip_gen",
                      "o_w1", "o_w2",
                      "o_w1T", "o_w2T", "o_w2p", "o_w2Tp", "o_w1Tp"):
                setattr(self, a, getattr(share_from, a))
            if self.E:
                self.o_wc = share_from.o_wc
        self._alloc_buffers()
        self.repack()

    def _build_params(self, seed):
        L, R, S, Kw, Cp, E = self.L, self.R, self.S, self.Kw, self.Cp, self.E
        secs: Dict[str, Section] = {}
        off = 0

        def add(name, shape):
            nonlocal off
            secs[name] = Section(name, off, shape)
            off += secs[name].numel

        add("init_w", (Kw, 1, R)); add("init_b", (R,))
        add("WF", (L, Kw, R, R)); add("BF", (L, R))
        if self.wavenet:
            add("WG", (L, Kw, R, R)); add("BG", (L, R))
        add("WR", (L, R, R)); add("BR", (L, R))
# ... 651 lines not shown
        los = [g[0] for g in self._wl_groups() if 0 < g[0] < self.L]
        return min(los, key=lambda v: abs(v - 0.4 * self.L)) if los else 0

    @property
    def contrastive(self) -> bool:
        return self.cfg.head_mode == "contrastive"

    @property
    def clip_head(self) -> bool:
        return self.cfg.head_mode in ("pooled", "contrastive")

    @property
    def bucket_off(self) -> int:
        return self.sections["WS"].offset

    @property
    def bucketed(self) -> bool:
        import os as _os
        forced = _os.environ.get("SRWN_FORCE_DIST") == "1"
        mode = _os.environ.get("SRWN_BUCKETS", "auto")
        if mode == "0" or not ((self.world > 1 or forced) and self.use_wl and self.split_layer > 0 and not self.clip_head):
            return False
        if mode == "1":
            return True
        import torch.distributed as dist
        return dist.is_initialized() and dist.get_backend(self.pg) == "nccl"

    def _bwd_head(self):
        B, T, N, S, Cp = self.B, self.T, self.N, self.S, self.Cp
        if self._head_bwd_done:
            return
        with _Span(self, "bwd_head"):
            if self.clip_head:
                from ._lib import call
                call("srwn_bcast_mask", self.dmean.data_ptr(), self.r1.data_ptr(), self.da1.data_ptr(), B, T, S,
                     1.0 / T, K.abi_dtype(self.dt), torch.cuda.current_stream().cuda_stream)
            else:
                K.pw_linear(self.dlogits.data_ptr(), Cp, 0, Cp, Cp, self.wptr(self.o_w2T), None, self.da1, S, S, N,
                            aux=self.r1, epi=K.EPI_MASK)
            K.pw_linear(self.da1.data_ptr(), S, 0, S, S, self.wptr(self.o_w1T), None, self.dtotal, S, S, N,
                        aux=self.r0, epi=K.EPI_MASK)

    def _wgrad_layers_group(self, l0: int, l1: int):
        N, L, R, T, ns = self.N, self.L, self.R, self.T, self.nslabs
        es = self.xs.element_size()
        NR = N * R
        ckw = {}
        with _Span(self, "wgrad_layers"):
            K.wgrad_layers(self.xs.view(L + 1, N, R)[l0:l1], self.zs.view(L, N, R)[l0:l1],
                           self.dfs.view(L, N, R)[l0:l1], self.gs.data_ptr() + (l0 + 1) * NR * es, self.dil[l0:l1],
                           self.pl_f[l0 * ns * 2 * R * R:], self.pl_r[l0 * ns * R * R:], self.pl_bf[l0 * ns * R:],
                           self.pl_br[l0 * ns * R:], T, ns, **ckw)

    def _wgrad_layers_finish(self):
        L, R, S, Kw, N, T = self.L, self.R, self.S, self.Kw, self.N, self.T
        gp, sec, ns, dt = self.grads.data_ptr(), self.sections, self.nslabs, self.dt
        es = self.xs.element_size()
        NR = N * R
        xs_p, dfs_p, gs_p = self.xs.data_ptr(), self.dfs.data_ptr(), self.gs.data_ptr()
        if self.use_wl:
            runs = []
            for (l0, l1), p16 in zip(self.groups, self.group_p16) if self.group_p16 else [((0, L), False)]:
                if runs and runs[-1][2] == p16:
                    runs[-1][1] = l1
                else:
                    runs.append([l0, l1, p16])
            jf, jr = [], []
            for l0, l1, p16 in runs:
                pl_f, pl_r = (self.pl_f, self.pl_r) if p16 or not self.part16 else (self.pl_f32, self.pl_r32)
                blk = (R,) if p16 else ()
                jf.append((pl_f[l0 * ns * Kw * R * R:], ns, Kw * R * R, l1 - l0, True, 1.0,
                           gp + 4 * (sec["WF"].offset + l0 * Kw * R * R), Kw * R * R) + blk)
                jr.append((pl_r[l0 * ns * R * R:], ns, R * R, l1 - l0, True, SQRT_HALF,
                           gp + 4 * (sec["WR"].offset + l0 * R * R), R * R) + blk)
            jobs = jf + [(self.pl_bf, ns, R, L, True, 1.0, gp + 4 * sec["BF"].offset, R)] + jr + [
                (self.pl_br, ns, R, L, True, SQRT_HALF, gp + 4 * sec["BR"].offset, R)]
            if self._ic_job is not None:
                jobs.append(self._ic_job)
                self._ic_job = None
            K.reduce_partials_multi(jobs)
            return
        if self.wavenet:
            self._wgrad_wavenet_convs()
        else:
            for k in range(Kw):
                shifts = [(Kw - 1 - k) * d for d in self.dil]
                last = k == Kw - 1
                K.wgrad(xs_p, NR, R, dfs_p, NR, R, shifts, L, self.wg_parts, self.wg_bparts if last else None, N, T, ns,
                        dt)
                K.reduce_partials(self.wg_parts, ns, R * R, L, True, 1.0, gp + 4 * (sec["WF"].offset + k * R * R),
                                  Kw * R * R)
                if last:
                    K.reduce_partials(self.wg_bparts, ns, R, L, True, 1.0, gp + 4 * sec["BF"].offset, R)
        K.wgrad(self._gate_out.data_ptr(), NR, R, gs_p + NR * es, NR, R, None, L, self.wg_parts, self.wg_bparts, N, T,
                ns, dt, pro=self._gate_pro)
        K.reduce_partials(self.wg_parts, ns, R * R, L, True, SQRT_HALF, gp + 4 * sec["WR"].offset, R * R)
        K.reduce_partials(self.wg_bparts, ns, R, L, True, SQRT_HALF, gp + 4 * sec["BR"].offset, R)

    def _wgrad_wavenet_convs(self):
        L, R, Kw, N, T, ns = self.L, self.R, self.Kw, self.N, self.T, self.nslabs
        NR = N * R
        for k in range(Kw):
            last = k == Kw - 1
            K.wgrad(self.xs.data_ptr(), NR, R, self.dfs.data_ptr(), 2 * NR, 2 * R, [(Kw - 1 - k) * d for d in self.dil], L,
                    self.wg_parts, self.wg_bparts if last else None, N, T, ns, self.dt)
            K.reduce_partials(self.wg_parts, ns, R * 2 * R, L, True, 1.0,
                              self.wn_wgrad.data_ptr() + 4 * k * R * 2 * R, Kw * R * 2 * R)
            if last:
                K.reduce_partials(self.wg_bparts, ns, 2 * R, L, True, 1.0, self.wn_bgrad.data_ptr(), 2 * R)
        g = self.grads
        self.view("WF", g).copy_(self.wn_wgrad[..., :R]); self.view("WG", g).copy_(self.wn_wgrad[..., R:])
        self.view("BF", g).copy_(self.wn_bgrad[:, :R]); self.view("BG", g).copy_(self.wn_bgrad[:, R:])

    def _wgrad_skip_and_head(self):
        N, T, L, R, S, Cp = self.N, self.T, self.L, self.R, self.S, self.Cp
        gp, sec, ns, dt = self.grads.data_ptr(), self.sections, self.nslabs, self.dt
        NR = N * R
        zs_p = self._gate_out.data_ptr()
        if self.batch_reduce:
            ns_skip = self.ns_skip
            with _Span(self, "wgrad_skip"):
                if self.skip_wt and self.fused_wt:
                    ns_skip = self.ns_skip_wt
                    K.wgrad_skip_wt(self.cTs, self.wt_layer_st, self.wt_layer_seg, self.dtotal,
                                    self.wg_parts if self.skip_parts16 is None else self.skip_parts16,
                                    self.wg_bparts, ns_skip, self.B, T, R)
                else:
                    K.wgrad256(zs_p, NR, R, L, self.dtotal, self.wg_parts, self.wg_bparts, N, self.ns_skip,
                               pro=self._gate_pro, chunk_width=R)
            if S == Cp:
                K.wgrad256_pair(self.r0.data_ptr(), self.da1, self.hd_parts[0], self.hd_bparts[0],
                                self.r1.data_ptr(), self.dlogits, self.hd_parts[1], self.hd_bparts[1], 64, S, S // 64, N,
                                self.ns_head)
            else:
                K.wgrad256(self.r0.data_ptr(), 64, S, S // 64, self.da1, self.hd_parts[0], self.hd_bparts[0], N, self.ns_head)
                K.wgrad256(self.r1.data_ptr(), 64, S, S // 64, self.dlogits, self.hd_parts[1], self.hd_bparts[1], N,
                           self.ns_head)
            skip16 = self.skip_wt and self.fused_wt and self.skip_parts16 is not None
            jobs = [
                (self.skip_parts16, ns_skip, L * R * S, 1, True, 1.0, gp + 4 * sec["WS"].offset, 0, S) if skip16 else
                (self.wg_parts, ns_skip, L * R * S, 1, True, 1.0, gp + 4 * sec["WS"].offset, 0),
                (self.wg_bparts, ns_skip, S, L, False, 1.0, gp + 4 * sec["BS"].offset, S),
                (self.hd_parts[0], self.ns_head, S * S, 1, True, 1.0, gp + 4 * sec["head_w1"].offset, 0),
                (self.hd_bparts[0], self.ns_head, S, 1, True, 1.0, gp + 4 * sec["head_b1"].offset, 0),
                (self.hd_parts[1], self.ns_head, S * Cp, 1, True, 1.0, gp + 4 * sec["head_w2"].offset, 0),
                (self.hd_bparts[1], self.ns_head, Cp, 1, True, 1.0, gp + 4 * sec["head_b2"].offset, 0)]
            if self._loss_job is not None:
                jobs.append(self._loss_job)
                self._loss_job = None
            K.reduce_partials_multi(jobs)
            return
        if self.use_w256:
            ns_skip = self.ns_skip
            with _Span(self, "wgrad_skip"):
                if self.skip_wt and self.fused_wt:
                    ns_skip = self.ns_skip_wt
                    K.wgrad_skip_wt(self.cTs, self.wt_layer_st, self.wt_layer_seg, self.dtotal,
                                    self.wg_parts if self.skip_parts16 is None else self.skip_parts16,
                                    self.wg_bparts, ns_skip, self.B, T, R)
                else:
                    K.wgrad256(zs_p, NR, R, L, self.dtotal, self.wg_parts, self.wg_bparts, N, self.ns_skip,
                               pro=self._gate_pro, chunk_width=R)
            if self.skip_wt and self.fused_wt and self.skip_parts16 is not None:
                K.reduce_partials_multi([(self.skip_parts16, ns_skip, L * R * S, 1, True, 1.0, gp + 4 * sec["WS"].offset, 0, S)])
            else:
                K.reduce_partials(self.wg_parts, ns_skip, L * R * S, 1, True, 1.0, gp + 4 * sec["WS"].offset, 0)
            K.reduce_partials(self.wg_bparts, ns_skip, S, L, False, 1.0, gp + 4 * sec["BS"].offset, S)
            K.wgrad256(self.r0.data_ptr(), 64, S, S // 64, self.da1, self.wg_parts, self.wg_bparts, N, self.ns_head)
            K.reduce_partials(self.wg_parts, self.ns_head, S * S, 1, True, 1.0, gp + 4 * sec["head_w1"].offset, 0)
            K.reduce_partials(self.wg_bparts, self.ns_head, S, 1, True, 1.0, gp + 4 * sec["head_b1"].offset, 0)
        else:
            with _Span(self, "wgrad_skip"):
                K.wgrad(zs_p, NR, R, self.dtotal.data_ptr(), 0, S, None, L, self.wg_parts, self.wg_bparts, N, T, ns,
                        dt, pro=self._gate_pro)
            K.reduce_partials(self.wg_parts, ns, R * S, L, True, 1.0, gp + 4 * sec["WS"].offset, R * S)
            K.reduce_partials(self.wg_bparts, ns, S, L, True, 1.0, gp + 4 * sec["BS"].offset, S)
            K.wgrad(self.r0.data_ptr(), 0, S, self.da1.data_ptr(), 0, S, None, 1, self.wg_parts, self.wg_bparts, N, T,
                    ns, dt)
            K.reduce_partials(self.wg_parts, ns, S * S, 1, True, 1.0, gp + 4 * sec["head_w1"].offset, 0)
            K.reduce_partials(self.wg_bparts, ns, S, 1, True, 1.0, gp + 4 * sec["head_b1"].offset, 0)
        if self.use_w256 and not self.clip_head and Cp == 256:
            K.wgrad256(self.r1.data_ptr(), 64, S, S // 64, self.dlogits, self.wg_parts, self.wg_bparts, N,
                       self.ns_head)
            K.reduce_partials(self.wg_parts, self.ns_head, S * Cp, 1, True, 1.0, gp + 4 * sec["head_w2"].offset, 0)
            K.reduce_partials(self.wg_bparts, self.ns_head, Cp, 1, True, 1.0, gp + 4 * sec["head_b2"].offset, 0)
        elif not self.clip_head:
            K.wgrad(self.r1.data_ptr(), 0, S, self.dlogits.data_ptr(), 0, Cp, None, 1, self.wg_parts, self.wg_bparts,
                    N, T, ns, dt)
            K.reduce_partials(self.wg_parts, ns, S * Cp, 1, True, 1.0, gp + 4 * sec["head_w2"].offset, 0)
            K.reduce_partials(self.wg_bparts, ns, Cp, 1, True, 1.0, gp + 4 * sec["head_b2"].offset, 0)

    def _wgrad_input_conv_partials(self):
        sec = self.sections
        assert sec["init_b"].offset == sec["init_w"].offset + sec["init_w"].numel
        nsl = K.init_conv_wgrad(self.audio, self.gs[0], None, None, self.Kw, 1 if self.cfg.shift_input else 0, self.ic_ws)
        self._ic_job = (self.ic_ws, nsl, (self.Kw + 1) * self.R, 1, True, 1.0,
                        self.grads.data_ptr() + 4 * sec["init_w"].offset, 0)

    def _wgrad_input_and_cond(self, input_conv: bool = True):
        B, T, L, R, Kw = self.B, self.T, self.L, self.R, self.Kw
        g = self.grads
        gp, sec, dt = g.data_ptr(), self.sections, self.dt
        if input_conv:
            K.init_conv_wgrad(self.audio, self.gs[0], self.view("init_w", g).reshape(-1), self.view("init_b", g), Kw,
                              1 if self.cfg.shift_input else 0, self.ic_ws)
        if self.E:
            rows_c, Ep, E = B * self.frames, self.Ep, self.E
            from ._lib import call
            call("srwn_frame_sum_batched", self.gs.data_ptr(), B * T * R, self.dcb.data_ptr(), rows_c * R, L, B, T, R,
                 self.frames, self.cfg.pool_stride, 1.0, K.abi_dtype(dt), torch.cuda.current_stream().cuda_stream)
            K.wgrad(self.cond_in.data_ptr(), 0, Ep, self.dcb.data_ptr(), rows_c * R, R, None, L, self.wgc_parts,
                    self.wgc_bparts, rows_c, self.frames, self.nslabs_c, dt)
            if Ep == E:
                K.reduce_partials(self.wgc_parts, self.nslabs_c, Ep * R, L, True, 1.0, gp + 4 * sec["WC"].offset, E * R)
            else:
                K.reduce_partials(self.wgc_parts, self.nslabs_c, Ep * R, L, True, 1.0, self.wc_grad_pad.data_ptr(),
                                  Ep * R)
                self.view("WC", g).copy_(self.wc_grad_pad[:, :E, :])
            K.reduce_partials(self.wgc_bparts, self.nslabs_c, R, L, True, 1.0, gp + 4 * sec["BC"].offset, R)

    def allreduce_grads(self):
        dp.allreduce_sum_(self.grads, self.pg)

    def optimizer_step(self):
        K.adam_step(self.params, self.grads, self.adam_m, self.adam_v, self.adam_step, self.cfg.learning_rate,
                    grad_scale=1.0 if self.mol else 1.0 / self.world)
        self.repack()

    def _allreduce_bucket_a(self):
        return dp.allreduce_sum_(self.grads[self.bucket_off:], self.pg, async_op=True)

    def _allreduce_bucket_b(self, pending):
        dp.allreduce_sum_(self.grads[:self.bucket_off], self.pg)
        if pending is not None:
            pending.wait()

    def train_step(self) -> torch.Tensor:
        self.forward(defer_loss=True)
        if self.bucketed and not self.timing:
            self.backward(part=1)
            h = self._allreduce_bucket_a()
            self.backward(part=2)
            self._allreduce_bucket_b(h)
        else:
            self.backward()
            self.allreduce_grads()
        self.optimizer_step()
        return self.loss

    def _check_generates(self):
        if self.wavenet:
            raise NotImplementedError("generate: gate_mode 'wavenet' is trained only; the generation kernels implement "
                                      "the reference gate (canonical generation is not built)")
        if self.o_gen is None or self.clip_head:
            raise NotImplementedError("generate: built for R=64 or 32, S=256 or 128, K=2 stacks with a per-time-step head")

    def _refuse_conditioned_softmax(self, cond=None):
        if not self.mol and (self.E or cond is not None):
            raise NotImplementedError("generate: the conditioned softmax teacher is not built (the conditioned "
                                      "decoder of the reference has the mixture-of-logistics head)")

    def _gen16(self) -> bool:
        return self.o_g16 is not None and _os.environ.get("SRWN_GEN16", "1") != "0"

    def _gen_dilations(self):
        return (ctypes.c_int32 * self.L)(*self.dil)

    def _gen_ring(self, n: int) -> torch.Tensor:
        from . import _lib
        relems = int(_lib.load().srwn_generate_ring_elems(self._gen_dilations(), self.L, self.R))
        return torch.zeros(relems * ((n + 31) // 32), dtype=self.dt, device=self.dev)

    def _gen_outputs(self, rows: int, nsteps: int, want_logits: bool, forced, rows_name: str = "batch"):
        audio = torch.zeros((rows, nsteps), dtype=torch.float32, device=self.dev)
        codes = torch.zeros((rows, nsteps), dtype=torch.int32, device=self.dev)
        logits = torch.zeros((rows, nsteps, self.C), dtype=torch.float32, device=self.dev) if want_logits else None
        if forced is not None:
            forced = torch.as_tensor(forced).to(device=self.dev, dtype=torch.float32).contiguous()
            if tuple(forced.shape) != (rows, nsteps):
                raise ValueError("forced must be [%s, nsteps]" % rows_name)
        return audio, codes, logits, forced

    def _project_cond(self, enc: torch.Tensor) -> torch.Tensor:
        rows, LR = enc.shape[0], self.L * self.R
        cin = torch.zeros((rows, self.Ep), dtype=self.dt, device=self.dev)
        cin[:, :self.E].copy_(enc)
        out = torch.empty((rows, LR), dtype=self.dt, device=self.dev)
        K.pw_linear(cin.data_ptr(), self.Ep, 0, self.Ep, self.Ep, self.wptr(self.o_wc), self.view("BC").reshape(-1), out,
                    LR, LR, rows)
        return out

# ... 152 lines not shown
            self._gen_prime_view = v
        return v

    def prime(self, state: "GenerationState", prompt: torch.Tensor) -> None:
        from . import _lib
        prompt = torch.as_tensor(prompt).to(device=self.dev, dtype=torch.float32)
        if prompt.dim() != 2 or prompt.shape[0] != state.batch:
            raise ValueError("prompt must be [batch=%d, P], got %s" % (state.batch, tuple(prompt.shape)))
        if state.t != 0:
            raise ValueError("prime: the state is at step %d; a prompt starts a run (t = 0)" % state.t)
        B, P = state.batch, int(prompt.shape[1])
        if state.limit is not None and P > state.limit:
            raise ValueError("prompt of %d samples exceeds frames * pool_stride = %d" % (P, state.limit))
        if P == 0:
            return
        pool = self.cfg.pool_stride if self.E else 1
        P_pad = -(-P // pool) * pool
        view = self._prime_view(B, P_pad)
        audio = torch.zeros((B, P_pad), dtype=torch.float32, device=self.dev)
        audio[:, :P].copy_(prompt)
        view.set_inputs(audio, None, state.cond[:, :P_pad // pool] if self.E else None)
        view.forward(want_logits=False, with_loss=False, train=False, stack_only=True)
        _lib.call("srwn_generate_ring_fill", view.xs.data_ptr(), B * P_pad * self.R, P_pad, P, self._gen_dilations(), self.L,
                  B, self.R, state.ring.data_ptr(), K.abi_dtype(self.dt), torch.cuda.current_stream().cuda_stream)
        state.carry[:, 0].copy_(prompt[:, P - 1])
        if P >= 2:
            state.carry[:, 1].copy_(prompt[:, P - 2])
        state.t = P

    def generate_chunk(self, state: "GenerationState", nsteps: int, mode: str = "sample",
                       forced: Optional[torch.Tensor] = None, want_logits: bool = False):
        B, nsteps = state.batch, int(nsteps)
        if nsteps < 0:
            raise ValueError("generate_chunk: nsteps %d" % nsteps)
        if state.limit is not None and state.t + nsteps > state.limit:
            raise ValueError("generate_chunk: steps %d..%d run past the encoding's frames * pool_stride = %d"
                             % (state.t, state.t + nsteps, state.limit))
        audio, codes, logits, forced = self._gen_outputs(B, nsteps, want_logits, forced)
        if nsteps == 0:
            return audio, codes, logits
        self._launch_generation(state.ring, audio, codes, logits, forced, B, nsteps, mode, state.seed, state.t, state.carry,
                                state.sampling, state.cond_all, state.frames, live=state.live)
        state.t += nsteps
        if state.live:
            state.cond = None
        return audio, codes, logits

    def capture_graphs(self):
        import os as _os
        torch.cuda.synchronize()
        self._g_fb = torch.cuda.CUDAGraph()
        self._g_b2 = None
        if self.world == 1 and _os.environ.get("SRWN_FORCE_DIST") != "1":
            with torch.cuda.graph(self._g_fb):
                self.forward(defer_loss=True)
                self.backward()
                self.optimizer_step()
            self._g_opt = None
            torch.cuda.synchronize()
            return
        with torch.cuda.graph(self._g_fb):
            self.forward(defer_loss=True)
            self.backward(part=1 if self.bucketed else 0)
        if self.bucketed:
            self._g_b2 = torch.cuda.CUDAGraph()
            with torch.cuda.graph(self._g_b2, pool=self._g_fb.pool()):
                self.backward(part=2)
        self._g_opt = torch.cuda.CUDAGraph()
        with torch.cuda.graph(self._g_opt, pool=self._g_fb.pool()):
            self.optimizer_step()
        torch.cuda.synchronize()

    def train_step_graphed(self) -> torch.Tensor:
        self._g_fb.replay()
        if self._g_opt is None:
            return self.loss
        if self._g_b2 is not None:
            h = self._allreduce_bucket_a()
            self._g_b2.replay()
            self._allreduce_bucket_b(h)
        else:
            self.allreduce_grads()
        self._g_opt.replay()
        return self.loss
```

sr-wavenet_amd/kernels.py:

```python
from __future__ import annotations

from typing import List, Optional, Tuple

import ctypes as _ct

import torch

from . import _lib
from ._lib import BF16, EPI_F32, EPI_MASK, EPI_NONE, EPI_RELU, F32, PRO_GATE, PRO_NONE, call

_TORCH2ABI = {torch.float32: F32, torch.bfloat16: BF16}


def abi_dtype(dt: torch.dtype) -> int:
    try:
        return _TORCH2ABI[dt]
    except KeyError:
        raise TypeError("unsupported activation dtype %s (float32 or bfloat16)" % dt)


def _stream() -> int:
    return torch.cuda.current_stream().cuda_stream


# ... 567 lines not shown
    if d0.shape != d1.shape or d0.shape[0] != rows or dw not in (128, 256):
        raise ValueError("wgrad256_pair: d0 %s d1 %s" % (tuple(d0.shape), tuple(d1.shape)))
    need = nslabs * m_chunks * chunk_width * dw
    for t, n in ((parts0, need), (parts1, need), (bparts0, nslabs * dw), (bparts1, nslabs * dw)):
        if t.numel() < n:
            raise ValueError("wgrad256_pair: partial buffer needs %d floats" % n)
    call("srwn_wgrad_wide_pair", a0_ptr, _chk(d0, "d0"), _chk(parts0, "partials0", torch.float32),
         _chk(bparts0, "bias_partials0", torch.float32), a1_ptr, _chk(d1, "d1"), _chk(parts1, "partials1", torch.float32),
         _chk(bparts1, "bias_partials1", torch.float32), int(a_chunk_stride), int(a_row_stride), int(m_chunks),
         int(chunk_width), dw, dw, int(rows), int(nslabs), PRO_NONE, abi_dtype(d0.dtype), _stream())


def _i32_array(vals):
    import ctypes as C
    return (C.c_int32 * len(vals))(*[int(v) for v in vals])


def wgrad_skip_wt_slabs(st, seg_rows, T: int) -> int:
    return int(_lib.load().srwn_wgrad_skip_wt_slabs(_i32_array(st), _i32_array(seg_rows), len(st), int(T)))


def wgrad_skip_wt(cT: torch.Tensor, st, seg_rows, d: torch.Tensor, partials: torch.Tensor,
                  bias_partials: Optional[torch.Tensor], nslabs: int, B: int, T: int, R: int):
    L = cT.shape[0]
    if len(st) != L or len(seg_rows) != L or d.shape[0] != B * T:
        raise ValueError("wgrad_skip_wt: %d layers, st %d, seg_rows %d, d %s" % (L, len(st), len(seg_rows), tuple(d.shape)))
    S = d.shape[-1]
    part16 = partials.dtype == torch.bfloat16
    pp = _chk(partials, "partials", torch.bfloat16 if part16 else torch.float32)
    if partials.numel() < nslabs * L * R * S:
        raise ValueError("wgrad_skip_wt: partials needs %d elements" % (nslabs * L * R * S))
    pb = None
    if bias_partials is not None:
        pb = _chk(bias_partials, "bias_partials", torch.float32)
        if bias_partials.numel() < nslabs * S:
            raise ValueError("wgrad_skip_wt: bias_partials needs %d floats" % (nslabs * S))
    call("srwn_wgrad_skip_wt", _chk(cT, "cT"), int(cT.stride(0)), _i32_array(st), _i32_array(seg_rows), L, _chk(d, "d"),
         int(d.stride(0)), pp, pb, 1 if part16 else 0, int(nslabs), int(B), int(T), int(R), int(S), abi_dtype(d.dtype),
         _stream())


def reduce_partials(partials: torch.Tensor, nslabs: int, n: int, nbatch: int, partials_batched: bool, scale: float,
                    out_ptr: int, out_batch_stride: int):
    call("srwn_reduce_partials", _chk(partials, "partials", torch.float32), int(nslabs), int(n), int(nbatch),
         int(bool(partials_batched)), float(scale), out_ptr, int(out_batch_stride), _stream())


class _ReduceJob(_ct.Structure):
    _fields_ = [("partials", _ct.c_void_p), ("nslabs", _ct.c_int32), ("n", _ct.c_int64), ("nbatch", _ct.c_int32),
                ("partials_batched", _ct.c_int32), ("scale", _ct.c_float), ("out", _ct.c_void_p),
                ("out_batch_stride", _ct.c_int64), ("layout", _ct.c_int32), ("blk_cols", _ct.c_int32)]


def reduce_partials_multi(jobs):
    arr = (_ReduceJob * len(jobs))()
    for j, job in zip(arr, jobs):
        partials, nslabs, n, nbatch, batched, scale, out_ptr, out_stride = job[:8]
        blk_cols = int(job[8]) if len(job) > 8 and job[8] != "sum" else 0
        j.partials = _chk(partials, "partials", torch.bfloat16 if blk_cols else torch.float32)
        j.layout, j.blk_cols = (1, blk_cols) if blk_cols else ((2, 0) if (len(job) > 8 and job[8] == "sum") else (0, 0))
        j.nslabs, j.n, j.nbatch, j.partials_batched = int(nslabs), int(n), int(nbatch), int(bool(batched))
        j.scale, j.out, j.out_batch_stride = float(scale), int(out_ptr), int(out_stride)
    call("srwn_reduce_partials_multi", _ct.addressof(arr), len(jobs), _stream())


def frame_sum(g: torch.Tensor, frames: int, pool_stride: int) -> torch.Tensor:
    B, T, Cc = g.shape
    out = torch.empty((B, frames, Cc), dtype=g.dtype, device=g.device)
    call("srwn_frame_sum", _chk(g, "g"), out.data_ptr(), B, T, Cc, int(frames), int(pool_stride), abi_dtype(g.dtype),
         _stream())
    return out


def adam_step(params: torch.Tensor, grads: torch.Tensor, m: torch.Tensor, v: torch.Tensor, step: torch.Tensor,
              lr: float, beta1: float = 0.9, beta2: float = 0.999, eps: float = 1e-8, grad_scale: float = 1.0):
    n = params.numel()
    for t, nm in ((params, "params"), (grads, "grads"), (m, "m"), (v, "v")):
        _chk(t, nm, torch.float32, (n,))
    _chk(step, "step", torch.int64, (1,))
    call("srwn_adam_step", params.data_ptr(), grads.data_ptr(), m.data_ptr(), v.data_ptr(), n, step.data_ptr(),
         float(lr), float(beta1), float(beta2), float(eps), float(grad_scale), _stream())


def flow_partials(rows: int) -> int:
    return int(_lib.load().srwn_flow_partials(int(rows)))


def flow_affine_fwd(h: torch.Tensor, w2: torch.Tensor, b2: torch.Tensor, x_in: torch.Tensor, prm: torch.Tensor,
                    x_out: torch.Tensor, ent_partials: torch.Tensor):
    rows, R = h.shape
    _chk(w2, "w2", torch.float32, (R, 2)); _chk(b2, "b2", torch.float32, (2,))
    _chk(x_in, "x_in", torch.float32, (rows,)); _chk(prm, "prm", torch.float32, (rows, 2))
    _chk(x_out, "x_out", torch.float32, (rows,))
    _chk(ent_partials, "ent_partials", torch.float32, (flow_partials(rows),))
    call("srwn_flow_affine_fwd", _chk(h, "h"), w2.data_ptr(), b2.data_ptr(), x_in.data_ptr(), prm.data_ptr(),
         x_out.data_ptr(), ent_partials.data_ptr(), rows, R, abi_dtype(h.dtype), _stream())


def flow_affine_bwd(h: torch.Tensor, w2: torch.Tensor, prm: torch.Tensor, x_in: torch.Tensor, dx_out: torch.Tensor,
                    ent_grad: float, g: torch.Tensor, dx_in: torch.Tensor, w_partials: torch.Tensor):
    rows, R = h.shape
    _chk(w2, "w2", torch.float32, (R, 2)); _chk(prm, "prm", torch.float32, (rows, 2))
    _chk(x_in, "x_in", torch.float32, (rows,)); _chk(dx_out, "dx_out", torch.float32, (rows,))
    _chk(g, "g", h.dtype, (rows, R)); _chk(dx_in, "dx_in", torch.float32, (rows,))
    _chk(w_partials, "w_partials", torch.float32, (flow_partials(rows), 2 * R + 2))
    call("srwn_flow_affine_bwd", _chk(h, "h"), w2.data_ptr(), prm.data_ptr(), x_in.data_ptr(), dx_out.data_ptr(),
         float(ent_grad), g.data_ptr(), dx_in.data_ptr(), w_partials.data_ptr(), rows, R, abi_dtype(h.dtype), _stream())


def causal_conv1d_dgrad(dy: torch.Tensor, w: torch.Tensor, dx: torch.Tensor, dilation: int = 1, shift: int = 0,
                        accumulate: bool = False, scale: float = 1.0):
    B, T, Cout = dy.shape
    K, Cin, Co2 = w.shape
    if Co2 != Cout:
        raise ValueError("causal_conv1d_dgrad: w %s vs dy %s" % (tuple(w.shape), tuple(dy.shape)))
    _chk(w, "w", torch.float32); _chk(dx, "dx", torch.float32, (B, T, Cin))
# ... 70 lines not shown
```

Before: 80.27 million samples/s.

## Fuse Adam update and param repacking into the gradient partial-reduction kernel

```diff
diff --git a/include/srwn.h b/include/srwn.h
--- a/include/srwn.h
+++ b/include/srwn.h
@@ -156,6 +156,14 @@
 
 int srwn_adam_step(float* params, const float* grads, float* m, float* v, int64_t n, int64_t* step, float lr,
                    float beta1, float beta2, float eps, float grad_scale, void* stream);
+
+#define SRWN_TAIL_ARRIVE_WORDS 1024
+int srwn_reduce_partials_adam(const SrwnReduceJob* jobs, int32_t njobs, const int32_t* job_is_param ,
+                              float* params, float* grads, float* m, float* v, int64_t nparams, int64_t* step,
+                              int32_t tick, float lr, float beta1, float beta2, float eps, float grad_scale,
+                              uint32_t* arrive, const int32_t* inv, int64_t inv_n, int32_t inv_fan, void* packed,
+                              int32_t dtype, const int32_t* gather_idx, int64_t gather_off, int64_t gather_n,
+                              const float* sum_src, int32_t sum_rows, int32_t sum_cols, float* sum_out, void* stream);
 
 int32_t srwn_time_mean_slabs(int32_t T);
 int srwn_time_mean(const void* x, float* partials, float* out, int32_t B, int32_t T, int32_t C, int32_t dtype,
diff --git a/sr-wavenet_amd/_lib.py b/sr-wavenet_amd/_lib.py
--- a/sr-wavenet_amd/_lib.py
+++ b/sr-wavenet_amd/_lib.py
@@ -206,7 +206,10 @@
 for _n in ("srwn_generate", "srwn_generate16"):
     SIGNATURES[_n + "_mol_live_sampled"] = SIGNATURES[_n + "_mol_resume_sampled"]
 del _n
-SIGNATURES["srwn_cond_ring_scatter"] = (C.c_int, [_p, _i64, _p, _i64, _i32, _i32, _i64, _i32, _i32, _i32, _p])
+SIGNATURES["srwn_reduce_partials_adam"] = (C.c_int, [_p, _i32, _p, _p, _p, _p, _p, _i64, _p, _i32, _f32, _f32, _f32, _f32,
+                                                     _f32, _p, _p, _i64, _i32, _p, _i32, _p, _i64, _i64, _p, _i32, _i32,
+                                                     _p, _p])
+SIGNATURES["srwn_cond_ring_scatter"] =(C.c_int, [_p, _i64, _p, _i64, _i32, _i32, _i64, _i32, _i32, _i32, _p])
 
 _lib = None
 BINDING = None
diff --git a/sr-wavenet_amd/csrc/srwn_bwd.hip b/sr-wavenet_amd/csrc/srwn_bwd.hip
--- a/sr-wavenet_amd/csrc/srwn_bwd.hip
+++ b/sr-wavenet_amd/csrc/srwn_bwd.hip
@@ -1,6 +1,7 @@
 #include <cstdlib>
 #include "srwn_common.h"
 #include "srwn_host.h"
+#include "srwn_tail.h"
 #include "../../include/srwn.h"
 
 using namespace srwn;
@@ -641,14 +642,16 @@
   int nslabs, nbatch, part_batch_mul; float scale; int wide; unsigned blocks_x, block0;
   int blk_cols;
   int sg;
+  int adam;
 };
 struct RpMulti { RpJob j[kRpMaxJobs]; int njobs; };
 
-__global__ __launch_bounds__(256) void reduce_partials_multi_kernel(RpMulti m) {
-  int k = 0;
-  while (k + 1 < m.njobs && blockIdx.x >= m.j[k + 1].block0) ++k;
-  const RpJob& job = m.j[k];
-  const unsigned b = blockIdx.x - job.block0;
+struct RpNoEpi {
+  template <int N> __device__ __forceinline__ void operator()(const float*, const float (&)[N]) const {}
+};
+
+template <typename Epi>
+__device__ __forceinline__ void rp_block(const RpJob& job, const unsigned b, const Epi& epi) {
   const unsigned bx = b % job.blocks_x;
   const int l = (int)(b / job.blocks_x);
   const int nslabs = job.nslabs;
@@ -684,6 +687,7 @@
         srwn::bf16x8 v[8];
 #pragma unroll
         for (int j = 0; j < 8; ++j) v[j] = SRWN_NT_LOAD(reinterpret_cast<const srwn::bf16x8*>(p + (int64_t)(k + j) * n));
+        __builtin_amdgcn_sched_barrier(0);
 #pragma unroll
         for (int j = 0; j < 8; ++j)
 #pragma unroll
@@ -719,7 +723,9 @@
 #pragma unroll
     for (int rr = 0; rr < 4; ++rr) {
       typedef float f2 __attribute__((ext_vector_type(2)));
-      *reinterpret_cast<f2*>(o + (int64_t)rr * job.blk_cols) = f2{(float)(s[rr] * sc), (float)(s[4 + rr] * sc)};
+      const float g2[2] = {(float)(s[rr] * sc), (float)(s[4 + rr] * sc)};
+      *reinterpret_cast<f2*>(o + (int64_t)rr * job.blk_cols) = f2{g2[0], g2[1]};
+      if (job.adam) epi(o + (int64_t)rr * job.blk_cols, g2);
     }
   } else if (job.wide == 1) {
     const int64_t i = (int64_t)bx * 16 + (threadIdx.x >> 4);
@@ -739,7 +745,11 @@
     }
 #pragma unroll
     for (int w = 8; w > 0; w >>= 1) s += __shfl_xor(s, w, 64);
-    if (i < n && sub == 0) job.out[(int64_t)l * job.out_batch_stride + i] = (float)(s * (double)job.scale);
+    if (i < n && sub == 0) {
+      const float g1[1] = {(float)(s * (double)job.scale)};
+      job.out[(int64_t)l * job.out_batch_stride + i] = g1[0];
+      if (job.adam) epi(job.out + (int64_t)l * job.out_batch_stride + i, g1);
+    }
   } else if (job.wide == 2) {
     const int64_t i = ((int64_t)bx * 256 + threadIdx.x) * 4;
     if (i >= n) return;
@@ -758,8 +768,9 @@
       s0 += (double)v[0]; s1 += (double)v[1]; s2 += (double)v[2]; s3 += (double)v[3];
     }
     const double sc = (double)job.scale;
-    *reinterpret_cast<srwn::f32x4*>(job.out + (int64_t)l * job.out_batch_stride + i) =
-        srwn::f32x4{(float)(s0 * sc), (float)(s1 * sc), (float)(s2 * sc), (float)(s3 * sc)};
+    const float g4[4] = {(float)(s0 * sc), (float)(s1 * sc), (float)(s2 * sc), (float)(s3 * sc)};
+    *reinterpret_cast<srwn::f32x4*>(job.out + (int64_t)l * job.out_batch_stride + i) = srwn::f32x4{g4[0], g4[1], g4[2], g4[3]};
+    if (job.adam) epi(job.out + (int64_t)l * job.out_batch_stride + i, g4);
   } else {
     const int64_t i = (int64_t)bx * 256 + threadIdx.x;
     if (i >= n) return;
@@ -774,24 +785,123 @@
       for (int j = 0; j < 8; ++j) s += (double)v[j];
     }
     for (; q < nslabs; ++q) s += (double)p[(int64_t)q * n];
-    job.out[(int64_t)l * job.out_batch_stride + i] = (float)(s * (double)job.scale);
-  }
-}
-
-extern "C" int srwn_reduce_partials_multi(const SrwnReduceJob* jobs, int32_t njobs, void* stream) {
-  if (njobs == 0) return 0;
-  if (!jobs) return set_error(SRWN_E_NULL, "reduce_partials_multi: null pointer");
-  if (njobs < 0 || njobs > kRpMaxJobs) return set_error(SRWN_E_SHAPE, "reduce_partials_multi: %d jobs (1..%d)", njobs, kRpMaxJobs);
-  RpMulti m;
+    const float g1[1] = {(float)(s * (double)job.scale)};
+    job.out[(int64_t)l * job.out_batch_stride + i] = g1[0];
+    if (job.adam) epi(job.out + (int64_t)l * job.out_batch_stride + i, g1);
+  }
+}
+
+__global__ __launch_bounds__(256) void reduce_partials_multi_kernel(RpMulti m) {
+  int k = 0;
+  while (k + 1 < m.njobs && blockIdx.x >= m.j[k + 1].block0) ++k;
+  rp_block(m.j[k], blockIdx.x - m.j[k].block0, RpNoEpi{});
+}
+
+struct TailEpi {
+  const float* grads; float* params; float* m; float* v;
+  float lr_t, b1, b2, eps, grad_scale;
+  const int32_t* inv; int64_t inv_n; int fan; void* packed; int dtype;
+  __device__ __forceinline__ void image(int32_t p, float th) const {
+    if (p < 0) return;
+    if (dtype == SRWN_BF16) reinterpret_cast<bf16_t*>(packed)[p] = (bf16_t)th;
+    else reinterpret_cast<float*>(packed)[p] = th;
+  }
+  template <int N> __device__ __forceinline__ void operator()(const float* o, const float (&g)[N]) const {
+    typedef float fN __attribute__((ext_vector_type(N)));
+    const int64_t i = o - grads;
+    float mm[N], vv[N], tt[N];
+    if constexpr (N == 1) {
+      mm[0] = m[i]; vv[0] = v[i]; tt[0] = params[i];
+    } else {
+      const fN a = *reinterpret_cast<const fN*>(m + i), b = *reinterpret_cast<const fN*>(v + i),
+               c = *reinterpret_cast<const fN*>(params + i);
+#pragma unroll
+      for (int j = 0; j < N; ++j) { mm[j] = a[j]; vv[j] = b[j]; tt[j] = c[j]; }
+    }
+#pragma unroll
+    for (int j = 0; j < N; ++j) adam_one(g[j], mm[j], vv[j], tt[j], grad_scale, lr_t, b1, b2, eps);
+    if constexpr (N == 1) {
+      m[i] = mm[0]; v[i] = vv[0]; params[i] = tt[0];
+    } else {
+      fN a, b, c;
+#pragma unroll
+      for (int j = 0; j < N; ++j) { a[j] = mm[j]; b[j] = vv[j]; c[j] = tt[j]; }
+      *reinterpret_cast<fN*>(m + i) = a; *reinterpret_cast<fN*>(v + i) = b; *reinterpret_cast<fN*>(params + i) = c;
+    }
+    if (!inv || i >= inv_n) return;
+    if (fan == 2) {
+      typedef int iN __attribute__((ext_vector_type(2 * N)));
+      const iN p = *reinterpret_cast<const iN*>(inv + 2 * i);
+#pragma unroll
+      for (int j = 0; j < N; ++j) { image(p[2 * j], tt[j]); image(p[2 * j + 1], tt[j]); }
+    } else {
+#pragma unroll
+      for (int j = 0; j < N; ++j)
+        for (int f = 0; f < fan; ++f) image(inv[(i + j) * fan + f], tt[j]);
+    }
+  }
+};
+
+struct RpTail {
+  const float* grads; float* params; float* m; float* v;
+  int64_t* step; unsigned* arrive; int tick;
+  float lr, b1, b2, eps, grad_scale;
+  const int32_t* inv; int64_t inv_n; int fan; void* packed; int dtype;
+  unsigned reduce_blocks, gather_blocks;
+  const int32_t* gidx; int64_t gather_off, gather_n;
+  const float* sum_src; int sum_rows, sum_cols; float* sum_out;
+};
+constexpr unsigned kTailGroups = SRWN_TAIL_ARRIVE_WORDS / 16;
+
+__global__ __launch_bounds__(256, 8) void reduce_partials_adam_kernel(RpMulti m, RpTail a) {
+  if (blockIdx.x >= a.reduce_blocks) {
+    const unsigned e = blockIdx.x - a.reduce_blocks;
+    if (e >= a.gather_blocks) {
+      column_sum_block(a.sum_src, a.sum_rows, a.sum_cols, a.sum_out, e - a.gather_blocks);
+    } else if (a.dtype == SRWN_BF16) {
+      pack_gather_block<bf16_t>(a.params, a.gidx, reinterpret_cast<bf16_t*>(a.packed) + a.gather_off, a.gather_n, e);
+    } else {
+      pack_gather_block<float>(a.params, a.gidx, reinterpret_cast<float*>(a.packed) + a.gather_off, a.gather_n, e);
+    }
+    return;
+  }
+  __shared__ float s_lr;
+  __shared__ int s_t;
+  if (threadIdx.x == 0) {
+    const int count = __hip_atomic_load(reinterpret_cast<int*>(a.step), __ATOMIC_RELAXED, __HIP_MEMORY_SCOPE_AGENT);
+    s_t = count + 1;
+    s_lr = adam_lr_t(a.lr, a.b1, a.b2, s_t);
+  }
+  __syncthreads();
+  const TailEpi epi{a.grads, a.params, a.m, a.v, s_lr, a.b1, a.b2, a.eps, a.grad_scale, a.inv, a.inv_n, a.fan, a.packed, a.dtype};
+  int k = 0;
+  while (k + 1 < m.njobs && blockIdx.x >= m.j[k + 1].block0) ++k;
+  rp_block(m.j[k], blockIdx.x - m.j[k].block0, epi);
+  if (a.tick && threadIdx.x == 0) {
+    const unsigned groups = a.reduce_blocks < kTailGroups ? a.reduce_blocks : kTailGroups;
+    const unsigned g = blockIdx.x % groups;
+    const unsigned members = a.reduce_blocks / groups + (g < a.reduce_blocks % groups ? 1u : 0u);
+    unsigned* word = a.arrive + 16 * g;
+    if (__hip_atomic_fetch_add(word, 1u, __ATOMIC_RELAXED, __HIP_MEMORY_SCOPE_AGENT) == members - 1) {
+      __hip_atomic_store(word, 0u, __ATOMIC_RELAXED, __HIP_MEMORY_SCOPE_AGENT);
+      unsigned* arrived = reinterpret_cast<unsigned*>(a.step) + 1;
+      if (__hip_atomic_fetch_add(arrived, 1u, __ATOMIC_RELAXED, __HIP_MEMORY_SCOPE_AGENT) == groups - 1)
+        __hip_atomic_store(a.step, (int64_t)s_t, __ATOMIC_RELAXED, __HIP_MEMORY_SCOPE_AGENT);
+    }
+  }
+}
+
+static int rp_setup(const SrwnReduceJob* jobs, int32_t njobs, RpMulti& m, uint64_t& blocks, const char* what) {
   m.njobs = 0;
-  uint64_t blocks = 0;
+  blocks = 0;
   for (int k = 0; k < njobs; ++k) {
     const SrwnReduceJob& q = jobs[k];
     if (q.n == 0 || q.nbatch == 0) continue;
-    if (!q.partials || !q.out) return set_error(SRWN_E_NULL, "reduce_partials_multi: job %d: null pointer", k);
+    if (!q.partials || !q.out) return set_error(SRWN_E_NULL, "%s: job %d: null pointer", what, k);
     if (q.nslabs < 1 || q.n < 0 || q.nbatch < 0 || q.nbatch > 65535)
-      return set_error(SRWN_E_SHAPE, "reduce_partials_multi: job %d: nslabs=%d n=%lld nbatch=%d", k, q.nslabs, (long long)q.n, q.nbatch);
+      return set_error(SRWN_E_SHAPE, "%s: job %d: nslabs=%d n=%lld nbatch=%d", what, k, q.nslabs, (long long)q.n, q.nbatch);
     RpJob& j = m.j[m.njobs++];
+    j.adam = 0;
     j.partials = reinterpret_cast<const float*>(q.partials); j.out = q.out; j.n = q.n; j.out_batch_stride = q.out_batch_stride;
     j.nslabs = q.nslabs; j.nbatch = q.nbatch; j.part_batch_mul = q.partials_batched ? 1 : 0; j.scale = q.scale;
     j.wide = (q.n <= 4096 && q.nslabs >= 32) ? 1 : 0;
@@ -802,24 +912,88 @@
     if (q.layout == SRWN_PARTIALS_BLK16) {
       if (q.blk_cols < 16 || q.blk_cols % 16 || q.n % (16 * (int64_t)q.blk_cols) || q.out_batch_stride % 2 ||
           (reinterpret_cast<uintptr_t>(q.partials) % 16) || (reinterpret_cast<uintptr_t>(q.out) % 8))
-        return set_error(SRWN_E_SHAPE, "reduce_partials_multi: job %d: BLK16 layout needs n = rows*blk_cols in whole 16 x 16 blocks (n=%lld, blk_cols=%d)", k, (long long)q.n, q.blk_cols);
+        return set_error(SRWN_E_SHAPE, "%s: job %d: BLK16 layout needs n = rows*blk_cols in whole 16 x 16 blocks (n=%lld, blk_cols=%d)", what, k, (long long)q.n, q.blk_cols);
       j.wide = 3; j.blk_cols = q.blk_cols;
       j.sg = 1;
       while (j.sg < 8 && q.nslabs / (2 * j.sg) >= 8 && (q.n / 8) * (int64_t)q.nbatch * j.sg < (int64_t)256 * 16 * 64) j.sg *= 2;
     } else if (q.layout == SRWN_PARTIALS_SUM) {
-      if (q.nbatch != 1) return set_error(SRWN_E_SHAPE, "reduce_partials_multi: job %d: SUM layout has one output", k);
+      if (q.nbatch != 1) return set_error(SRWN_E_SHAPE, "%s: job %d: SUM layout has one output", what, k);
       j.wide = 4;
     } else if (q.layout != SRWN_PARTIALS_F32) {
-      return set_error(SRWN_E_UNSUPPORTED, "reduce_partials_multi: job %d: layout %d", k, q.layout);
+      return set_error(SRWN_E_UNSUPPORTED, "%s: job %d: layout %d", what, k, q.layout);
     }
     j.blocks_x = (unsigned)(j.wide == 4 ? 1 : j.wide == 3 ? (q.n / 8 + 256 / j.sg - 1) / (256 / j.sg) : j.wide == 2 ? (q.n / 4 + 255) / 256 : j.wide ? (q.n + 15) / 16 : (q.n + 255) / 256);
     j.block0 = (unsigned)blocks;
     blocks += (uint64_t)j.blocks_x * (uint64_t)q.nbatch;
-    if (blocks > 0x7fffffffull) return set_error(SRWN_E_SHAPE, "reduce_partials_multi: grid too large");
-  }
+    if (blocks > 0x7fffffffull) return set_error(SRWN_E_SHAPE, "%s: grid too large", what);
+  }
+  return 0;
+}
+
+extern "C" int srwn_reduce_partials_multi(const SrwnReduceJob* jobs, int32_t njobs, void* stream) {
+  if (njobs == 0) return 0;
+  if (!jobs) return set_error(SRWN_E_NULL, "reduce_partials_multi: null pointer");
+  if (njobs < 0 || njobs > kRpMaxJobs) return set_error(SRWN_E_SHAPE, "reduce_partials_multi: %d jobs (1..%d)", njobs, kRpMaxJobs);
+  RpMulti m;
+  uint64_t blocks;
+  if (const int rc = rp_setup(jobs, njobs, m, blocks, "reduce_partials_multi")) return rc;
   if (m.njobs == 0) return 0;
   hipLaunchKernelGGL(reduce_partials_multi_kernel, dim3((unsigned)blocks), dim3(256), 0, (hipStream_t)stream, m);
   return check_launch("reduce_partials_multi");
+}
+
+extern "C" int srwn_reduce_partials_adam(const SrwnReduceJob* jobs, int32_t njobs, const int32_t* job_is_param,
+                                         float* params, float* grads, float* m, float* v, int64_t nparams, int64_t* step,
+                                         int32_t tick, float lr, float beta1, float beta2, float eps, float grad_scale,
+                                         uint32_t* arrive, const int32_t* inv, int64_t inv_n, int32_t inv_fan,
+                                         void* packed, int32_t dtype, const int32_t* gather_idx, int64_t gather_off,
+                                         int64_t gather_n, const float* sum_src, int32_t sum_rows, int32_t sum_cols,
+                                         float* sum_out, void* stream) {
+  const char* what = "reduce_partials_adam";
+  if (njobs < 0 || njobs > kRpMaxJobs) return set_error(SRWN_E_SHAPE, "%s: %d jobs (0..%d)", what, njobs, kRpMaxJobs);
+  if ((njobs && (!jobs || !job_is_param)) || !params || !grads || !m || !v || !step || !arrive)
+    return set_error(SRWN_E_NULL, "%s: null pointer", what);
+  const bool sum = sum_rows > 0 && sum_cols > 0;
+  if (nparams < 0 || nparams > 0x7fffffffll || inv_n < 0 || inv_n > nparams || inv_fan < 0 || gather_off < 0 || gather_n < 0 ||
+      sum_rows < 0 || sum_cols < 0)
+    return set_error(SRWN_E_SHAPE, "%s: nparams=%lld inv_n=%lld fan=%d gather=[%lld,+%lld) sum %d x %d", what, (long long)nparams,
+                     (long long)inv_n, inv_fan, (long long)gather_off, (long long)gather_n, sum_rows, sum_cols);
+  if ((((uintptr_t)params) | ((uintptr_t)grads) | ((uintptr_t)m) | ((uintptr_t)v) | ((uintptr_t)inv) | ((uintptr_t)arrive)) & 15)
+    return set_error(SRWN_E_SHAPE, "%s: params, grads, m, v, inv and arrive must be 16-byte aligned", what);
+  if ((inv || gather_n) && dtype != SRWN_F32 && dtype != SRWN_BF16) return set_error(SRWN_E_DTYPE, "%s: dtype %d", what, dtype);
+  if ((inv || gather_n) && !packed) return set_error(SRWN_E_NULL, "%s: null image", what);
+  if (gather_n && (!gather_idx || (((uintptr_t)gather_idx) & 15) ||
+                   (((uintptr_t)packed + (uintptr_t)gather_off * (dtype == SRWN_BF16 ? 2 : 4)) & 15)))
+    return set_error(SRWN_E_SHAPE, "%s: the gathered range and its index must be 16-byte aligned", what);
+  if (sum && (!sum_src || !sum_out)) return set_error(SRWN_E_NULL, "%s: null column-sum pointer", what);
+  RpMulti jm;
+  uint64_t blocks;
+  if (const int rc = rp_setup(jobs, njobs, jm, blocks, what)) return rc;
+  for (int k = 0, kk = 0; k < njobs; ++k) {
+    const SrwnReduceJob& q = jobs[k];
+    if (q.n == 0 || q.nbatch == 0) continue;
+    RpJob& j = jm.j[kk++];
+    j.adam = job_is_param[k] ? 1 : 0;
+    if (!j.adam) continue;
+    const int64_t lo = q.out - grads, hi = lo + (int64_t)(q.nbatch - 1) * q.out_batch_stride + q.n;
+    if (q.layout == SRWN_PARTIALS_SUM || q.out_batch_stride < 0 || lo < 0 || hi > nparams)
+      return set_error(SRWN_E_SHAPE, "%s: job %d is marked a parameter gradient but does not write grads[0, %lld)", what, k, (long long)nparams);
+    if (inv && inv_fan > 0 && lo < inv_n && hi > inv_n)
+      return set_error(SRWN_E_SHAPE, "%s: job %d straddles the end of the inverse index (%lld)", what, k, (long long)inv_n);
+  }
+  if (tick && blocks == 0) return set_error(SRWN_E_SHAPE, "%s: tick = 1 needs a job (the reduction's blocks advance the step)", what);
+  if (blocks == 0 && gather_n == 0 && !sum) return 0;
+  RpTail a;
+  a.grads = grads; a.params = params; a.m = m; a.v = v; a.step = step; a.arrive = arrive; a.tick = tick ? 1 : 0;
+  a.lr = lr; a.b1 = beta1; a.b2 = beta2; a.eps = eps; a.grad_scale = grad_scale;
+  a.inv = inv_fan > 0 ? inv : nullptr; a.inv_n = inv_n; a.fan = inv_fan; a.packed = packed; a.dtype = dtype;
+  a.reduce_blocks = (unsigned)blocks; a.gather_blocks = (unsigned)((gather_n + 2047) / 2048);
+  a.gidx = gather_idx; a.gather_off = gather_off; a.gather_n = gather_n;
+  a.sum_src = sum_src; a.sum_rows = sum ? sum_rows : 0; a.sum_cols = sum ? sum_cols : 0; a.sum_out = sum_out;
+  const uint64_t grid = blocks + a.gather_blocks + (sum ? (uint64_t)(sum_cols + 255) / 256 : 0);
+  if (grid > 0x7fffffffull) return set_error(SRWN_E_SHAPE, "%s: grid too large", what);
+  hipLaunchKernelGGL(reduce_partials_adam_kernel, dim3((unsigned)grid), dim3(256), 0, (hipStream_t)stream, jm, a);
+  return check_launch(what);
 }
 
 extern "C" int srwn_reduce_partials(const float* partials, int32_t nslabs, int64_t n, int32_t nbatch,
diff --git a/sr-wavenet_amd/csrc/srwn_opt.hip b/sr-wavenet_amd/csrc/srwn_opt.hip
--- a/sr-wavenet_amd/csrc/srwn_opt.hip
+++ b/sr-wavenet_amd/csrc/srwn_opt.hip
@@ -1,5 +1,6 @@
 #include "srwn_common.h"
 #include "srwn_host.h"
+#include "srwn_tail.h"
 #include "../../include/srwn.h"
 
 using namespace srwn;
@@ -23,18 +24,12 @@
   if (threadIdx.x == 0) {
     const int count = __hip_atomic_load(reinterpret_cast<int*>(step), __ATOMIC_RELAXED, __HIP_MEMORY_SCOPE_AGENT);
     s_t = count + (tick ? 1 : 0);
-    const double t = (double)s_t;
-    s_lr = (float)((double)lr * sqrt(1.0 - pow((double)b2, t)) / (1.0 - pow((double)b1, t)));
+    s_lr = adam_lr_t(lr, b1, b2, s_t);
   }
   __syncthreads();
   const float lr_t = s_lr;
   if (scale_dev) grad_scale *= scale_dev[0];
-  auto one = [&](float gi, float& mi, float& vi, float& th) {
-    gi *= grad_scale;
-    mi = b1 * mi + (1.0f - b1) * gi;
-    vi = b2 * vi + (1.0f - b2) * gi * gi;
-    th -= lr_t * mi / (sqrtf(vi) + eps);
-  };
+  auto one = [&](float gi, float& mi, float& vi, float& th) { adam_one(gi, mi, vi, th, grad_scale, lr_t, b1, b2, eps); };
   for (int64_t i0 = ((int64_t)blockIdx.x * blockDim.x + threadIdx.x) * 4; i0 < n; i0 += (int64_t)gridDim.x * blockDim.x * 4) {
     if (vec && i0 + 4 <= n) {
       typedef float f4 __attribute__((ext_vector_type(4)));
diff --git a/sr-wavenet_amd/csrc/srwn_pybind.cpp b/sr-wavenet_amd/csrc/srwn_pybind.cpp
--- a/sr-wavenet_amd/csrc/srwn_pybind.cpp
+++ b/sr-wavenet_amd/csrc/srwn_pybind.cpp
@@ -11,7 +11,7 @@
 
 PYBIND11_MODULE(_srwn_pyb, m) {
   m.doc() = "pybind11 binding of libsrwn.so (include/srwn.h)";
-  m.attr("SIGNATURE_HASH") = "921a0d5f5da475ed";
+  m.attr("SIGNATURE_HASH") = "9ff97db7d3b4595c";
   m.def("srwn_version", []() { return srwn_version(); });
   m.def("srwn_last_error", []() { const char* r = srwn_last_error(); return py::bytes(r ? r : ""); });
   m.def("srwn_mu_law_encode", [](std::uintptr_t a0, std::uintptr_t a1, int64_t a2, int a3, std::uintptr_t a4) { return srwn_mu_law_encode(P{a0}, P{a1}, a2, a3, P{a4}); });
@@ -143,5 +143,6 @@
   m.def("srwn_generate16_mol_slots_sampled", [](std::uintptr_t a0, std::uintptr_t a1, std::uintptr_t a2, std::uintptr_t a3, std::uintptr_t a4, std::uintptr_t a5, std::uintptr_t a6, std::uintptr_t a7, std::uintptr_t a8, std::uintptr_t a9, std::uintptr_t a10, std::uintptr_t a11, std::uintptr_t a12, std::uintptr_t a13, std::uintptr_t a14, std::uintptr_t a15, int a16, int a17, int a18, int a19, int a20, int a21, int a22, std::uintptr_t a23, int a24, int a25, int64_t a26, int a27, std::uintptr_t a28, int a29, std::uintptr_t a30, std::uintptr_t a31, std::uintptr_t a32) { return srwn_generate16_mol_slots_sampled(P{a0}, P{a1}, P{a2}, P{a3}, P{a4}, P{a5}, P{a6}, P{a7}, P{a8}, P{a9}, P{a10}, P{a11}, P{a12}, P{a13}, P{a14}, P{a15}, a16, a17, a18, a19, a20, a21, a22, P{a23}, a24, a25, a26, a27, P{a28}, a29, P{a30}, P{a31}, P{a32}); });
   m.def("srwn_generate_mol_live_sampled", [](std::uintptr_t a0, std::uintptr_t a1, std::uintptr_t a2, std::uintptr_t a3, std::uintptr_t a4, std::uintptr_t a5, std::uintptr_t a6, std::uintptr_t a7, std::uintptr_t a8, std::uintptr_t a9, std::uintptr_t a10, std::uintptr_t a11, std::uintptr_t a12, std::uintptr_t a13, std::uintptr_t a14, std::uintptr_t a15, std::uintptr_t a16, int a17, int a18, int a19, int a20, int a21, int a22, int a23, int a24, std::uintptr_t a25, int a26, int a27, int64_t a28, int a29, uint64_t a30, int a31, std::uintptr_t a32, int a33, std::uintptr_t a34, std::uintptr_t a35) { return srwn_generate_mol_live_sampled(P{a0}, P{a1}, P{a2}, P{a3}, P{a4}, P{a5}, P{a6}, P{a7}, P{a8}, P{a9}, P{a10}, P{a11}, P{a12}, P{a13}, P{a14}, P{a15}, P{a16}, a17, a18, a19, a20, a21, a22, a23, a24, P{a25}, a26, a27, a28, a29, a30, a31, P{a32}, a33, P{a34}, P{a35}); });
   m.def("srwn_generate16_mol_live_sampled", [](std::uintptr_t a0, std::uintptr_t a1, std::uintptr_t a2, std::uintptr_t a3, std::uintptr_t a4, std::uintptr_t a5, std::uintptr_t a6, std::uintptr_t a7, std::uintptr_t a8, std::uintptr_t a9, std::uintptr_t a10, std::uintptr_t a11, std::uintptr_t a12, std::uintptr_t a13, std::uintptr_t a14, std::uintptr_t a15, int a16, int a17, int a18, int a19, int a20, int a21, int a22, std::uintptr_t a23, int a24, int a25, int64_t a26, int a27, uint64_t a28, std::uintptr_t a29, int a30, std::uintptr_t a31, std::uintptr_t a32) { return srwn_generate16_mol_live_sampled(P{a0}, P{a1}, P{a2}, P{a3}, P{a4}, P{a5}, P{a6}, P{a7}, P{a8}, P{a9}, P{a10}, P{a11}, P{a12}, P{a13}, P{a14}, P{a15}, a16, a17, a18, a19, a20, a21, a22, P{a23}, a24, a25, a26, a27, a28, P{a29}, a30, P{a31}, P{a32}); });
+  m.def("srwn_reduce_partials_adam", [](std::uintptr_t a0, int a1, std::uintptr_t a2, std::uintptr_t a3, std::uintptr_t a4, std::uintptr_t a5, std::uintptr_t a6, int64_t a7, std::uintptr_t a8, int a9, float a10, float a11, float a12, float a13, float a14, std::uintptr_t a15, std::uintptr_t a16, int64_t a17, int a18, std::uintptr_t a19, int a20, std::uintptr_t a21, int64_t a22, int64_t a23, std::uintptr_t a24, int a25, int a26, std::uintptr_t a27, std::uintptr_t a28) { return srwn_reduce_partials_adam(P{a0}, a1, P{a2}, P{a3}, P{a4}, P{a5}, P{a6}, a7, P{a8}, a9, a10, a11, a12, a13, a14, P{a15}, P{a16}, a17, a18, P{a19}, a20, P{a21}, a22, a23, P{a24}, a25, a26, P{a27}, P{a28}); });
   m.def("srwn_cond_ring_scatter", [](std::uintptr_t a0, int64_t a1, std::uintptr_t a2, int64_t a3, int a4, int a5, int64_t a6, int a7, int a8, int a9, std::uintptr_t a10) { return srwn_cond_ring_scatter(P{a0}, a1, P{a2}, a3, a4, a5, a6, a7, a8, a9, P{a10}); });
 }
diff --git a/sr-wavenet_amd/csrc/srwn_tail.h b/sr-wavenet_amd/csrc/srwn_tail.h
--- /dev/null
+++ b/sr-wavenet_amd/csrc/srwn_tail.h
@@ -0,0 +1,57 @@
+#pragma once
+#include "srwn_common.h"
+
+namespace srwn {
+
+__device__ __forceinline__ float adam_lr_t(float lr, float b1, float b2, int t_int) {
+  const double t = (double)t_int;
+  return (float)((double)lr * sqrt(1.0 - pow((double)b2, t)) / (1.0 - pow((double)b1, t)));
+}
+
+__device__ __forceinline__ void adam_one(float gi, float& mi, float& vi, float& th, float grad_scale, float lr_t,
+                                         float b1, float b2, float eps) {
+  gi *= grad_scale;
+  mi = b1 * mi + (1.0f - b1) * gi;
+  vi = b2 * vi + (1.0f - b2) * gi * gi;
+  th -= lr_t * mi / (sqrtf(vi) + eps);
+}
+
+template <typename T>
+__device__ __forceinline__ void pack_gather_block(const float* __restrict__ src, const int32_t* __restrict__ idx,
+                                                  T* __restrict__ dst, int64_t n, unsigned blk) {
+  const int64_t i0 = ((int64_t)blk * 256 + threadIdx.x) * 8;
+  if (i0 >= n) return;
+  if (i0 + 8 <= n) {
+    typedef int i32x4 __attribute__((ext_vector_type(4)));
+    const i32x4 a = *reinterpret_cast<const i32x4*>(idx + i0), b = *reinterpret_cast<const i32x4*>(idx + i0 + 4);
+    float v[8];
+#pragma unroll
+    for (int j = 0; j < 4; ++j) { v[j] = a[j] >= 0 ? src[a[j]] : 0.0f; v[4 + j] = b[j] >= 0 ? src[b[j]] : 0.0f; }
+    if constexpr (sizeof(T) == 2) {
+      bf16x8 o;
+#pragma unroll
+      for (int j = 0; j < 8; ++j) o[j] = (bf16_t)v[j];
+      *reinterpret_cast<bf16x8*>(dst + i0) = o;
+    } else {
+      *reinterpret_cast<f32x4*>(dst + i0) = f32x4{v[0], v[1], v[2], v[3]};
+      *reinterpret_cast<f32x4*>(dst + i0 + 4) = f32x4{v[4], v[5], v[6], v[7]};
+    }
+  } else {
+    for (int64_t i = i0; i < n; ++i) {
+      const int32_t s = idx[i];
+      dst[i] = (T)(s >= 0 ? src[s] : 0.0f);
+    }
+  }
+}
+
+__device__ __forceinline__ void column_sum_block(const float* __restrict__ sum_src, int sum_rows, int sum_cols,
+                                                 float* __restrict__ sum_out, unsigned blk) {
+  const int c = (int)blk * 256 + (int)threadIdx.x;
+  if (c < sum_cols) {
+    double s = 0.0;
+    for (int l = 0; l < sum_rows; ++l) s += (double)sum_src[(size_t)l * sum_cols + c];
+    sum_out[c] = (float)s;
+  }
+}
+
+}
diff --git a/sr-wavenet_amd/csrc/srwn_util.hip b/sr-wavenet_amd/csrc/srwn_util.hip
--- a/sr-wavenet_amd/csrc/srwn_util.hip
+++ b/sr-wavenet_amd/csrc/srwn_util.hip
@@ -1,5 +1,6 @@
 #include "srwn_common.h"
 #include "srwn_host.h"
+#include "srwn_tail.h"
 #include "../../include/srwn.h"
 
 using namespace srwn;
@@ -20,7 +21,7 @@
 }
 }
 
-extern "C" int srwn_version(void) { return 112; }
+extern "C" int srwn_version(void) { return 113; }
 extern "C" const char* srwn_last_error(void) { return g_err; }
 
 __global__ void mu_law_encode_kernel(const float* __restrict__ audio, int32_t* __restrict__ codes, int64_t n,
@@ -108,37 +109,10 @@
                                                           const float* __restrict__ sum_src, int sum_rows, int sum_cols,
                                                           float* __restrict__ sum_out) {
   if (blockIdx.x >= gather_blocks) {
-    const int c = (int)(blockIdx.x - gather_blocks) * 256 + (int)threadIdx.x;
-    if (c < sum_cols) {
-      double s = 0.0;
-      for (int l = 0; l < sum_rows; ++l) s += (double)sum_src[(size_t)l * sum_cols + c];
-      sum_out[c] = (float)s;
-    }
+    column_sum_block(sum_src, sum_rows, sum_cols, sum_out, blockIdx.x - gather_blocks);
     return;
   }
-  const int64_t i0 = ((int64_t)blockIdx.x * blockDim.x + threadIdx.x) * 8;
-  if (i0 >= n) return;
-  if (i0 + 8 <= n) {
-    typedef int i32x4 __attribute__((ext_vector_type(4)));
-    const i32x4 a = *reinterpret_cast<const i32x4*>(idx + i0), b = *reinterpret_cast<const i32x4*>(idx + i0 + 4);
-    float v[8];
-#pragma unroll
-    for (int j = 0; j < 4; ++j) { v[j] = a[j] >= 0 ? src[a[j]] : 0.0f; v[4 + j] = b[j] >= 0 ? src[b[j]] : 0.0f; }
-    if constexpr (sizeof(T) == 2) {
-      bf16x8 o;
-#pragma unroll
-      for (int j = 0; j < 8; ++j) o[j] = (bf16_t)v[j];
-      *reinterpret_cast<bf16x8*>(dst + i0) = o;
-    } else {
-      *reinterpret_cast<f32x4*>(dst + i0) = f32x4{v[0], v[1], v[2], v[3]};
-      *reinterpret_cast<f32x4*>(dst + i0 + 4) = f32x4{v[4], v[5], v[6], v[7]};
-    }
-  } else {
-    for (int64_t i = i0; i < n; ++i) {
-      const int32_t s = idx[i];
-      dst[i] = (T)(s >= 0 ? src[s] : 0.0f);
-    }
-  }
+  pack_gather_block<T>(src, idx, dst, n, blockIdx.x);
 }
 
 extern "C" int srwn_pack_gather_rowsum(const float* src, const int32_t* idx, void* dst, int64_t n, int32_t dtype,
diff --git a/sr-wavenet_amd/engine.py b/sr-wavenet_amd/engine.py
--- a/sr-wavenet_amd/engine.py
+++ b/sr-wavenet_amd/engine.py
@@ -388,6 +388,8 @@
                            and cfg.dtype == torch.bfloat16 and cfg.skip_channels == 256)
         self._head_bwd_done = False
         self._ic_job = None
+        self._tail = None
+        self._tail_on = False
         self._loss_job = None
         self.defer_loss = _os.environ.get("SRWN_DEFER_LOSS", "1") != "0"
         self.side = None
@@ -1145,6 +1147,26 @@
                            self.pl_f[l0 * ns * 2 * R * R:], self.pl_r[l0 * ns * R * R:], self.pl_bf[l0 * ns * R:],
                            self.pl_br[l0 * ns * R:], T, ns, **ckw)
 
+    def _layer_jobs(self):
+        L, R, Kw = self.L, self.R, self.Kw
+        gp, sec, ns = self.grads.data_ptr(), self.sections, self.nslabs
+        runs = []
+        for (l0, l1), p16 in zip(self.groups, self.group_p16) if self.group_p16 else [((0, L), False)]:
+            if runs and runs[-1][2] == p16:
+                runs[-1][1] = l1
+            else:
+                runs.append([l0, l1, p16])
+        jf, jr = [], []
+        for l0, l1, p16 in runs:
+            pl_f, pl_r = (self.pl_f, self.pl_r) if p16 or not self.part16 else (self.pl_f32, self.pl_r32)
+            blk = (R,) if p16 else ()
+            jf.append((pl_f[l0 * ns * Kw * R * R:], ns, Kw * R * R, l1 - l0, True, 1.0,
+                       gp + 4 * (sec["WF"].offset + l0 * Kw * R * R), Kw * R * R) + blk)
+            jr.append((pl_r[l0 * ns * R * R:], ns, R * R, l1 - l0, True, SQRT_HALF,
+                       gp + 4 * (sec["WR"].offset + l0 * R * R), R * R) + blk)
+        return jf + [(self.pl_bf, ns, R, L, True, 1.0, gp + 4 * sec["BF"].offset, R)] + jr + [
+            (self.pl_br, ns, R, L, True, SQRT_HALF, gp + 4 * sec["BR"].offset, R)]
+
     def _wgrad_layers_finish(self):
         L, R, S, Kw, N, T = self.L, self.R, self.S, self.Kw, self.N, self.T
         gp, sec, ns, dt = self.grads.data_ptr(), self.sections, self.nslabs, self.dt
@@ -1152,26 +1174,11 @@
         NR = N * R
         xs_p, dfs_p, gs_p = self.xs.data_ptr(), self.dfs.data_ptr(), self.gs.data_ptr()
         if self.use_wl:
-            runs = []
-            for (l0, l1), p16 in zip(self.groups, self.group_p16) if self.group_p16 else [((0, L), False)]:
-                if runs and runs[-1][2] == p16:
-                    runs[-1][1] = l1
-                else:
-                    runs.append([l0, l1, p16])
-            jf, jr = [], []
-            for l0, l1, p16 in runs:
-                pl_f, pl_r = (self.pl_f, self.pl_r) if p16 or not self.part16 else (self.pl_f32, self.pl_r32)
-                blk = (R,) if p16 else ()
-                jf.append((pl_f[l0 * ns * Kw * R * R:], ns, Kw * R * R, l1 - l0, True, 1.0,
-                           gp + 4 * (sec["WF"].offset + l0 * Kw * R * R), Kw * R * R) + blk)
-                jr.append((pl_r[l0 * ns * R * R:], ns, R * R, l1 - l0, True, SQRT_HALF,
-                           gp + 4 * (sec["WR"].offset + l0 * R * R), R * R) + blk)
-            jobs = jf + [(self.pl_bf, ns, R, L, True, 1.0, gp + 4 * sec["BF"].offset, R)] + jr + [
-                (self.pl_br, ns, R, L, True, SQRT_HALF, gp + 4 * sec["BR"].offset, R)]
+            jobs = self._layer_jobs()
             if self._ic_job is not None:
                 jobs.append(self._ic_job)
                 self._ic_job = None
-            K.reduce_partials_multi(jobs)
+            self._finish_jobs(jobs, last=True)
             return
         if self.wavenet:
             self._wgrad_wavenet_convs()
@@ -1204,6 +1211,20 @@
         g = self.grads
         self.view("WF", g).copy_(self.wn_wgrad[..., :R]); self.view("WG", g).copy_(self.wn_wgrad[..., R:])
         self.view("BF", g).copy_(self.wn_bgrad[:, :R]); self.view("BG", g).copy_(self.wn_bgrad[:, R:])
+
+    def _skip_head_jobs(self):
+        L, R, S, Cp = self.L, self.R, self.S, self.Cp
+        gp, sec = self.grads.data_ptr(), self.sections
+        ns_skip = self.ns_skip_wt if (self.skip_wt and self.fused_wt) else self.ns_skip
+        skip16 = self.skip_wt and self.fused_wt and self.skip_parts16 is not None
+        return [
+            (self.skip_parts16, ns_skip, L * R * S, 1, True, 1.0, gp + 4 * sec["WS"].offset, 0, S) if skip16 else
+            (self.wg_parts, ns_skip, L * R * S, 1, True, 1.0, gp + 4 * sec["WS"].offset, 0),
+            (self.wg_bparts, ns_skip, S, L, False, 1.0, gp + 4 * sec["BS"].offset, S),
+            (self.hd_parts[0], self.ns_head, S * S, 1, True, 1.0, gp + 4 * sec["head_w1"].offset, 0),
+            (self.hd_bparts[0], self.ns_head, S, 1, True, 1.0, gp + 4 * sec["head_b1"].offset, 0),
+            (self.hd_parts[1], self.ns_head, S * Cp, 1, True, 1.0, gp + 4 * sec["head_w2"].offset, 0),
+            (self.hd_bparts[1], self.ns_head, Cp, 1, True, 1.0, gp + 4 * sec["head_b2"].offset, 0)]
 
     def _wgrad_skip_and_head(self):
         N, T, L, R, S, Cp = self.N, self.T, self.L, self.R, self.S, self.Cp
@@ -1229,19 +1250,11 @@
                 K.wgrad256(self.r0.data_ptr(), 64, S, S // 64, self.da1, self.hd_parts[0], self.hd_bparts[0], N, self.ns_head)
                 K.wgrad256(self.r1.data_ptr(), 64, S, S // 64, self.dlogits, self.hd_parts[1], self.hd_bparts[1], N,
                            self.ns_head)
-            skip16 = self.skip_wt and self.fused_wt and self.skip_parts16 is not None
-            jobs = [
-                (self.skip_parts16, ns_skip, L * R * S, 1, True, 1.0, gp + 4 * sec["WS"].offset, 0, S) if skip16 else
-                (self.wg_parts, ns_skip, L * R * S, 1, True, 1.0, gp + 4 * sec["WS"].offset, 0),
-                (self.wg_bparts, ns_skip, S, L, False, 1.0, gp + 4 * sec["BS"].offset, S),
-                (self.hd_parts[0], self.ns_head, S * S, 1, True, 1.0, gp + 4 * sec["head_w1"].offset, 0),
-                (self.hd_bparts[0], self.ns_head, S, 1, True, 1.0, gp + 4 * sec["head_b1"].offset, 0),
-                (self.hd_parts[1], self.ns_head, S * Cp, 1, True, 1.0, gp + 4 * sec["head_w2"].offset, 0),
-                (self.hd_bparts[1], self.ns_head, Cp, 1, True, 1.0, gp + 4 * sec["head_b2"].offset, 0)]
+            jobs = self._skip_head_jobs()
             if self._loss_job is not None:
                 jobs.append(self._loss_job)
                 self._loss_job = None
-            K.reduce_partials_multi(jobs)
+            self._finish_jobs(jobs, last=False)
             return
         if self.use_w256:
             ns_skip = self.ns_skip
@@ -1315,6 +1328,71 @@
     def allreduce_grads(self):
         dp.allreduce_sum_(self.grads, self.pg)
 
+    def _tail_plan(self):
+        if self._tail is not None:
+            return self._tail or None
+        self._tail = False
+        ok = (self.world == 1 and self.use_wl and getattr(self, "batch_reduce", False) and self.fused_wt
+              and not self.E and not self.wavenet and not self.clip_head and not self.frozen
+              and getattr(self, "bs_sum", None) is not None and "BS" in self.sections and self.fused_bwd)
+        if not ok:
+            return None
+        off, n, cut, stop = self.bucket_off, self.nparams, self.o_skipT_all, self.pack_train_elems
+        g0 = self.grads.data_ptr() // 4
+        sec = self.sections
+        ic = (None, 1, (self.Kw + 1) * self.R, 1, True, 1.0, self.grads.data_ptr() + 4 * sec["init_w"].offset, 0)
+
+        def tiles(jobs, lo, hi):
+            spans = sorted(r for j in jobs for r in K.job_outputs(j))
+            at = g0 + lo
+            for a, b in spans:
+                if a != at or b <= a:
+                    return False
+                at = b
+            return at == g0 + hi
+        if not (tiles(self._skip_head_jobs(), off, n) and tiles(self._layer_jobs() + [ic], 0, off)):
+            return None
+        pk = self.packer
+        if getattr(pk, "tail_inv", None) is None:
+            idx = pk.idx[:stop].cpu().numpy()
+            lower, upper = idx[:cut], idx[cut:]
+            if (lower >= off).any() or ((upper >= 0) & (upper < off)).any() or cut % 8 or (stop - cut) % 8:
+                return None
+            inv, fan = K.inverse_gather_index(lower, off)
+            pk.tail_inv = (torch.from_numpy(inv).to(self.dev), off, fan)
+            pk.tail_arrive = torch.zeros(K.TAIL_ARRIVE_WORDS, dtype=torch.int32, device=self.dev)
+        self._tail = {"inv": pk.tail_inv, "arrive": pk.tail_arrive, "cut": cut, "stop": stop}
+        return self._tail
+
+    def _tail_fused(self) -> bool:
+        if _os.environ.get("SRWN_FUSE_TAIL", "1") == "0" or _os.environ.get("SRWN_FORCE_DIST") == "1":
+            return False
+        return self._tail_plan() is not None
+
+    def _finish_jobs(self, jobs, last: bool):
+        if not self._tail_on:
+            K.reduce_partials_multi(jobs)
+            return
+        tp = self._tail
+        flags = [not (len(j) > 8 and j[8] == "sum") for j in jobs]
+        scatter = _os.environ.get("SRWN_TAIL_SCATTER", "1") != "0"
+        kw = {}
+        if last:
+            kw = dict(inv=tp["inv"] if scatter else None, packed=self.packed,
+                      gather=(self.packer.idx[tp["cut"]:], tp["cut"], tp["stop"] - tp["cut"]),
+                      rowsum=(self.view("BS"), self.bs_sum))
+        K.reduce_partials_adam(jobs, flags, self.params, self.grads, self.adam_m, self.adam_v, self.adam_step, last,
+                               self.cfg.learning_rate, tp["arrive"], grad_scale=1.0, **kw)
+        if last and not scatter:
+            self.packer.gather(self.params, self.packed, 0, tp["cut"])
+
+    def _backward_and_update(self):
+        self._tail_on = True
+        try:
+            self.backward()
+        finally:
+            self._tail_on = False
+
     def optimizer_step(self):
         K.adam_step(self.params, self.grads, self.adam_m, self.adam_v, self.adam_step, self.cfg.learning_rate,
                     grad_scale=1.0 if self.mol else 1.0 / self.world)
@@ -1330,6 +1408,9 @@
 
     def train_step(self) -> torch.Tensor:
         self.forward(defer_loss=True)
+        if self._tail_fused():
+            self._backward_and_update()
+            return self.loss
         if self.bucketed and not self.timing:
             self.backward(part=1)
             h = self._allreduce_bucket_a()
@@ -1588,10 +1669,14 @@
         self._g_fb = torch.cuda.CUDAGraph()
         self._g_b2 = None
         if self.world == 1 and _os.environ.get("SRWN_FORCE_DIST") != "1":
+            fused = self._tail_fused()
             with torch.cuda.graph(self._g_fb):
                 self.forward(defer_loss=True)
-                self.backward()
-                self.optimizer_step()
+                if fused:
+                    self._backward_and_update()
+                else:
+                    self.backward()
+                    self.optimizer_step()
             self._g_opt = None
             torch.cuda.synchronize()
             return
diff --git a/sr-wavenet_amd/kernels.py b/sr-wavenet_amd/kernels.py
--- a/sr-wavenet_amd/kernels.py
+++ b/sr-wavenet_amd/kernels.py
@@ -643,7 +643,7 @@
                 ("out_batch_stride", _ct.c_int64), ("layout", _ct.c_int32), ("blk_cols", _ct.c_int32)]
 
 
-def reduce_partials_multi(jobs):
+def _reduce_jobs(jobs):
     arr = (_ReduceJob * len(jobs))()
     for j, job in zip(arr, jobs):
         partials, nslabs, n, nbatch, batched, scale, out_ptr, out_stride = job[:8]
@@ -652,7 +652,73 @@
         j.layout, j.blk_cols = (1, blk_cols) if blk_cols else ((2, 0) if (len(job) > 8 and job[8] == "sum") else (0, 0))
         j.nslabs, j.n, j.nbatch, j.partials_batched = int(nslabs), int(n), int(nbatch), int(bool(batched))
         j.scale, j.out, j.out_batch_stride = float(scale), int(out_ptr), int(out_stride)
+    return arr
+
+
+def reduce_partials_multi(jobs):
+    arr = _reduce_jobs(jobs)
     call("srwn_reduce_partials_multi", _ct.addressof(arr), len(jobs), _stream())
+
+
+TAIL_ARRIVE_WORDS = 1024
+
+
+def job_outputs(job):
+    n, nbatch, out_ptr, out_stride = int(job[2]), int(job[3]), int(job[6]), int(job[7])
+    n = 1 if (len(job) > 8 and job[8] == "sum") else n
+    return [(out_ptr // 4 + l * out_stride, out_ptr // 4 + l * out_stride + n) for l in range(nbatch)]
+
+
+def inverse_gather_index(idx, n_src: int):
+    import numpy as np
+    idx = np.asarray(idx).reshape(-1).astype(np.int64)
+    pos = np.nonzero(idx >= 0)[0]
+    src = idx[pos]
+    if src.size and int(src.max()) >= n_src:
+        raise ValueError("inverse_gather_index: the index reads source %d of %d" % (int(src.max()), n_src))
+    counts = np.bincount(src, minlength=n_src)
+    fan = int(counts.max()) if src.size else 0
+    inv = np.full(n_src * max(fan, 1), -1, dtype=np.int32)
+    order = np.argsort(src, kind="stable")
+    src_s, pos_s = src[order], pos[order]
+    first = np.concatenate([[0], np.cumsum(counts)[:-1]])
+    rank = np.arange(src_s.size) - first[src_s]
+    inv[src_s * fan + rank] = pos_s
+    return inv, fan
+
+
+def reduce_partials_adam(jobs, is_param, params: torch.Tensor, grads: torch.Tensor, m: torch.Tensor, v: torch.Tensor,
+                         step: torch.Tensor, tick: bool, lr: float, arrive: torch.Tensor, beta1: float = 0.9,
+                         beta2: float = 0.999, eps: float = 1e-8, grad_scale: float = 1.0, inv=None, packed=None,
+                         gather=None, rowsum=None):
+    n = params.numel()
+    for t, nm in ((params, "params"), (grads, "grads"), (m, "m"), (v, "v")):
+        _chk(t, nm, torch.float32, (n,))
+    _chk(step, "step", torch.int64, (1,))
+    _chk(arrive, "arrive", torch.int32, (TAIL_ARRIVE_WORDS,))
+    if len(is_param) != len(jobs):
+        raise ValueError("reduce_partials_adam: one is_param flag per job")
+    arr = _reduce_jobs(jobs)
+    flags = (_ct.c_int32 * max(len(jobs), 1))(*[int(bool(f)) for f in is_param])
+    inv_p, inv_n, fan = (None, 0, 0) if inv is None else (_chk(inv[0], "inv", torch.int32), int(inv[1]), int(inv[2]))
+    if inv is not None and inv[0].numel() < inv_n * fan:
+        raise ValueError("reduce_partials_adam: inv holds %d entries, %d x %d needed" % (inv[0].numel(), inv_n, fan))
+    g_p, g_off, g_n = (None, 0, 0) if gather is None else (_chk(gather[0], "gather index", torch.int32), int(gather[1]),
+                                                           int(gather[2]))
+    if gather is not None and (gather[0].numel() < g_n or packed is None or g_off + g_n > packed.numel()):
+        raise ValueError("reduce_partials_adam: gather of [%d, +%d)" % (g_off, g_n))
+    if inv is not None and packed is None:
+        raise ValueError("reduce_partials_adam: inv without an image")
+    s_p, s_rows, s_cols, s_out = None, 0, 0, None
+    if rowsum is not None:
+        mat, vec = rowsum
+        s_p = _chk(mat, "rowsum matrix", torch.float32)
+        s_out = _chk(vec, "rowsum out", torch.float32, (mat.shape[-1],))
+        s_rows, s_cols = int(mat.numel() // mat.shape[-1]), int(mat.shape[-1])
+    call("srwn_reduce_partials_adam", _ct.addressof(arr), len(jobs), _ct.addressof(flags), params.data_ptr(), grads.data_ptr(),
+         m.data_ptr(), v.data_ptr(), n, step.data_ptr(), int(bool(tick)), float(lr), float(beta1), float(beta2), float(eps),
+         float(grad_scale), arrive.data_ptr(), inv_p, inv_n, fan, None if packed is None else packed.data_ptr(),
+         abi_dtype(packed.dtype) if packed is not None else 0, g_p, g_off, g_n, s_p, s_rows, s_cols, s_out, _stream())
 
 
 def frame_sum(g: torch.Tensor, frames: int, pool_stride: int) -> torch.Tensor:
```

Result: no change. 80.49 million samples/s, median of 6 (+0.3%).
